# megaease/easevoice-trainer

Measured on AMD Instinct MI355X. Metric: audio-seconds/sec trained (s2), higher is better.
Workload: dtype bf16; 1 GPU; s2 SoVITS generator+discriminator GAN step, batch=16/GPU, 4 s 32 kHz clips (T=200 frames), configs/s2.json, random-init weights; global_batch=16, parallelism=dp1, launch=hip-graph replay (3 graphs/step)

## Files before the change

easevoice_trainer_amd/csrc/wn_layer.hip:

```cpp
#include "resunit_common.h"
#include "../../include/evt.h"
#include <type_traits>

namespace {

using namespace evt_ru;

struct WNP {
  const h16_t* x;
  const h16_t* w_in;
  const h16_t* w_rs;
  const float* b_in;
  const float* b_rs;
  const h16_t* g;
  const h16_t* acc_in;
  const int* lens;
  h16_t* x_in;
  h16_t* acts;
  h16_t* x_out;
  h16_t* acc_out;
  int nseq, L, tps;
};

__device__ __forceinline__ float sigmoid_f(float x) {
  return __builtin_amdgcn_rcpf(1.f + __builtin_amdgcn_exp2f(x * -1.4426950408889634f));
}
__device__ __forceinline__ float tanh_f(float x) { return fmaf(2.f, sigmoid_f(2.f * x), -1.f); }

__device__ __forceinline__ int wslot(int row, int slot) { return slot ^ (row & 7); }

__device__ __forceinline__ void unpack4(const u32x2 v, float (&o)[4]) {
  o[0] = h2f_lo(v[0]); o[1] = h2f_hi(v[0]);
  o[2] = h2f_lo(v[1]); o[3] = h2f_hi(v[1]);
}

template <int H, int K, int NT, int R, bool LAST>
__global__ __launch_bounds__(256, 1) void wn_layer_fwd(WNP p) {
  constexpr int PITCH = H * 2;
  constexpr int SPR = H / 8;
  constexpr int NCH = H / 32;
  constexpr int MT = H / 16 / 4;
  constexpr int P = 16 * NT;
  constexpr int HALO = (K - 1) / 2;
  constexpr int XROWS = P + K - 1;
  constexpr int NKA = NCH * K, NKB = NCH;
  constexpr int MA = 2 * MT;
  constexpr int MB = LAST ? MT : 2 * MT;
  static_assert(H % 64 == 0 && SPR % 8 == 0, "rows of whole 128-byte groups, M-tiles divisible by the four waves");
  extern __shared__ __attribute__((aligned(1024))) unsigned char smem[];
  unsigned char* xs = smem;
  unsigned char* acl = smem + ((XROWS + 7) & ~7) * PITCH;
  const int tid = threadIdx.x, lane = tid & 63, wm = __builtin_amdgcn_readfirstlane(tid >> 6);
  const int n = lane & 15, g = lane >> 4;
  const int seq = blockIdx.x / p.tps;
  const int q0 = (blockIdx.x - seq * p.tps) * P;
  const long sbase = (long)seq * p.L;

  u32x4 fa[R][MA];
  auto tileA = [&](int i) {
    return i < MT ? wm * MT + i : H / 16 + wm * MT + i - MT;
  };
  auto issue_a = [&](const h16_t* w, const int nk, const int ks, const int s, auto cnt) {
    constexpr int CNT = decltype(cnt)::value;
#pragma unroll
    for (int i = 0; i < CNT; ++i)
      fa[s][i] = *reinterpret_cast<const u32x4*>(w + ((long)(tileA(i) * nk + ks) * 64 + lane) * 8);
  };
  using CA = std::integral_constant<int, MA>;
  using CB = std::integral_constant<int, MB>;

  constexpr int NP = XROWS * SPR;
  constexpr int PER = (NP + 255) / 256;
  uint4 xv[PER];
#pragma unroll
  for (int u = 0; u < PER; ++u) {
    const int idx = u * 256 + tid;
    const int r = idx / SPR, sl = idx - r * SPR;
    const int pos = q0 - HALO + r;
    xv[u] = (idx < NP && pos >= 0 && pos < p.L) ? *reinterpret_cast<const uint4*>(p.x + (sbase + pos) * H + sl * 8)
                                                : make_uint4(0, 0, 0, 0);
  }
#pragma unroll
  for (int s = 0; s < R - 1 && s < NKA; ++s) issue_a(p.w_in, NKA, s, s, CA{});
  float bA0[MT][4], bA1[MT][4], bB0[MT][4], bB1[MT][4];
  u32x2 gA0[MT], gA1[MT], accp[MT][NT];
  const int len = p.lens ? p.lens[seq] : p.L;
#pragma unroll
  for (int i = 0; i < MT; ++i) {
    const int h = (wm * MT + i) * 16 + g * 4;
    const f32x4 z = {0.f, 0.f, 0.f, 0.f};
    const f32x4 a0 = p.b_in ? *reinterpret_cast<const f32x4*>(p.b_in + h) : z;
    const f32x4 a1 = p.b_in ? *reinterpret_cast<const f32x4*>(p.b_in + H + h) : z;
    const f32x4 c0 = p.b_rs ? *reinterpret_cast<const f32x4*>(p.b_rs + h) : z;
    const f32x4 c1 = (!LAST && p.b_rs) ? *reinterpret_cast<const f32x4*>(p.b_rs + H + h) : z;
#pragma unroll
    for (int r = 0; r < 4; ++r) { bA0[i][r] = a0[r]; bA1[i][r] = a1[r]; bB0[i][r] = c0[r]; bB1[i][r] = c1[r]; }
    gA0[i] = gA1[i] = u32x2{0u, 0u};
    if (p.g) {
      gA0[i] = *reinterpret_cast<const u32x2*>(p.g + (long)seq * 2 * H + h);
      gA1[i] = *reinterpret_cast<const u32x2*>(p.g + (long)seq * 2 * H + H + h);
    }
#pragma unroll
    for (int j = 0; j < NT; ++j) {
      const int pos = q0 + j * 16 + n;
      accp[i][j] = (p.acc_in && pos < p.L) ? *reinterpret_cast<const u32x2*>(p.acc_in + (sbase + pos) * H + h) : u32x2{0u, 0u};
    }
  }
#pragma unroll
  for (int u = 0; u < PER; ++u) {
    const int idx = u * 256 + tid;
    if (idx >= NP) continue;
    const int r = idx / SPR, sl = idx - r * SPR;
    *reinterpret_cast<uint4*>(xs + r * PITCH + wslot(r, sl) * 16) = xv[u];
  }
  __syncthreads();

  auto conv = [&](auto& acc, const h16_t* w, auto nk_c, auto taps_c, auto cnt, const unsigned char* rows) {
    constexpr int NK = decltype(nk_c)::value, TAPS = decltype(taps_c)::value, CNT = decltype(cnt)::value;
    u32x4 fb[NT];
    auto b_addr = [&](const int ks) {
      const int ch = ks / TAPS, tap = ks - ch * TAPS;
      const int row = n + tap;
      return rows + row * PITCH + wslot(row, ch * 4 + g) * 16;
    };
    {
      const unsigned char* b0 = b_addr(0);
#pragma unroll
      for (int j = 0; j < NT; ++j) {
        fb[j] = *reinterpret_cast<const u32x4*>(b0 + j * 16 * PITCH);
      }
    }
#pragma unroll
    for (int ks = 0; ks < NK; ++ks) {
      const int s = ks % R;
      if (ks + R - 1 < NK) issue_a(w, NK, ks + R - 1, (ks + R - 1) % R, cnt);
#pragma unroll
      for (int i = 0; i < CNT; ++i) tie(fa[s][i]);
      const unsigned char* nb = b_addr(ks + 1 < NK ? ks + 1 : ks);
#pragma unroll
      for (int j = 0; j < NT; ++j) {
        tie(fb[j]);
#pragma unroll
        for (int i = 0; i < CNT; ++i)
          acc[i][j] = EVT_MFMA_16x16x32(as_h8(fa[s][i]), as_h8(fb[j]), acc[i][j], 0, 0, 0);
        fb[j] = *reinterpret_cast<const u32x4*>(nb + j * 16 * PITCH);
      }
    }
  };

  {
    f32x4 acc[MA][NT];
#pragma unroll
    for (int i = 0; i < MA; ++i)
#pragma unroll
      for (int j = 0; j < NT; ++j) acc[i][j] = f32x4{0.f, 0.f, 0.f, 0.f};
    conv(acc, p.w_in, std::integral_constant<int, NKA>{}, std::integral_constant<int, K>{}, CA{}, xs);
#pragma unroll
    for (int s = 0; s < R - 1 && s < NKB; ++s) issue_a(p.w_rs, NKB, s, s, CB{});
#pragma unroll
    for (int i = 0; i < MT; ++i) {
      const int h = (wm * MT + i) * 16 + g * 4;
      float ga[4], gb[4];
      unpack4(gA0[i], ga);
      unpack4(gA1[i], gb);
#pragma unroll
      for (int j = 0; j < NT; ++j) {
        const int m = j * 16 + n;
        const int pos = q0 + m;
        h16_t xa[4], xb[4], o4[4];
#pragma unroll
        for (int r = 0; r < 4; ++r) {
          xa[r] = f2h(acc[i][j][r] + bA0[i][r]);
          xb[r] = f2h(acc[MT + i][j][r] + bA1[i][r]);
          const float a = h2f(xa[r]) + ga[r], b = h2f(xb[r]) + gb[r];
          o4[r] = f2h(tanh_f(a) * sigmoid_f(b));
        }
        *reinterpret_cast<uint2*>(acl + m * PITCH + wslot(m, h >> 3) * 16 + (h & 7) * 2) = *reinterpret_cast<uint2*>(o4);
        if (pos < p.L) {
          h16_t* xi = p.x_in + (sbase + pos) * 2 * H + h;
          *reinterpret_cast<uint2*>(xi) = *reinterpret_cast<uint2*>(xa);
          *reinterpret_cast<uint2*>(xi + H) = *reinterpret_cast<uint2*>(xb);
          *reinterpret_cast<uint2*>(p.acts + (sbase + pos) * H + h) = *reinterpret_cast<uint2*>(o4);
        }
      }
    }
  }
  __syncthreads();

  {
    f32x4 acc[MB][NT];
#pragma unroll
    for (int i = 0; i < MB; ++i)
#pragma unroll
      for (int j = 0; j < NT; ++j) acc[i][j] = f32x4{0.f, 0.f, 0.f, 0.f};
    conv(acc, p.w_rs, std::integral_constant<int, NKB>{}, std::integral_constant<int, 1>{}, CB{}, acl);
#pragma unroll
    for (int i = 0; i < MT; ++i) {
      const int h = (wm * MT + i) * 16 + g * 4;
#pragma unroll
      for (int j = 0; j < NT; ++j) {
        const int m = j * 16 + n;
        const int pos = q0 + m;
        if (pos >= p.L) continue;
        const bool live = pos < len;
        float ap[4];
        unpack4(accp[i][j], ap);
        h16_t o1[4], o2[4];
        if constexpr (LAST) {
#pragma unroll
          for (int r = 0; r < 4; ++r) {
            const float rs = h2f(f2h(acc[i][j][r] + bB0[i][r]));
            o2[r] = f2h(live ? ap[r] + rs : 0.f);
          }
        } else {
          float xo[4];
          const int xr = HALO + m;
          unpack4(*reinterpret_cast<const u32x2*>(xs + xr * PITCH + wslot(xr, h >> 3) * 16 + (h & 7) * 2), xo);
#pragma unroll
          for (int r = 0; r < 4; ++r) {
            const float r0 = h2f(f2h(acc[i][j][r] + bB0[i][r]));
            const float r1 = h2f(f2h(acc[MT + i][j][r] + bB1[i][r]));
            o1[r] = f2h(live ? xo[r] + r0 : 0.f);
            o2[r] = f2h(ap[r] + r1);
          }
          *reinterpret_cast<uint2*>(p.x_out + (sbase + pos) * H + h) = *reinterpret_cast<uint2*>(o1);
        }
        *reinterpret_cast<uint2*>(p.acc_out + (sbase + pos) * H + h) = *reinterpret_cast<uint2*>(o2);
      }
    }
  }
}

struct WNB {
  const h16_t* dx_next;
  const h16_t* dacc;
  const h16_t* x_in;
  const h16_t* g;
  const h16_t* w_rs;
  const h16_t* w_in;
  const int* lens;
  h16_t* drs;
  h16_t* dx_in;
  h16_t* dx;
  float* dg;
  int nseq, L, tps;
};

__device__ __forceinline__ int wslot2(int row, int slot) { return slot ^ ((row & 7) << 1); }

__device__ __forceinline__ float sum16(float v) {
  v += __shfl_xor(v, 1, 16);
  v += __shfl_xor(v, 2, 16);
  v += __shfl_xor(v, 4, 16);
  v += __shfl_xor(v, 8, 16);
  return v;
}

template <int H, int K, int NT, int R, bool LAST>
__global__ __launch_bounds__(256, 1) void wn_layer_bwd(WNB p) {
  constexpr int PB = H * 4;
  constexpr int SPRB = H / 4;
  constexpr int MT = H / 16 / 4;
  constexpr int P = 16 * NT;
  constexpr int HALO = (K - 1) / 2;
  constexpr int NT1 = NT + 1;
  constexpr int ROWS = P + 2 * HALO;
  constexpr int CIN1 = LAST ? H : 2 * H;
  constexpr int NK1 = CIN1 / 32, NK2 = (2 * H / 32) * K;
  static_assert(2 * HALO <= 16, "one extra position tile covers the halo");
  extern __shared__ __attribute__((aligned(1024))) unsigned char smem[];
  unsigned char* ds = smem;
  unsigned char* es = smem + 16 * NT1 * PB;
  const int tid = threadIdx.x, lane = tid & 63, wm = __builtin_amdgcn_readfirstlane(tid >> 6);
  const int n = lane & 15, g = lane >> 4;
  const int seq = blockIdx.x / p.tps;
  const int q0 = (blockIdx.x - seq * p.tps) * P;
  const long sbase = (long)seq * p.L;
  const int len = p.lens ? p.lens[seq] : p.L;

  u32x4 fa[R][MT];
  auto issue_a = [&](const h16_t* w, const int nk, const int ks, const int s) {
#pragma unroll
    for (int i = 0; i < MT; ++i)
      fa[s][i] = *reinterpret_cast<const u32x4*>(w + ((long)((wm * MT + i) * nk + ks) * 64 + lane) * 8);
  };

  constexpr int SPR1 = CIN1 / 8;
  constexpr int NP = ROWS * SPR1;
  constexpr int PER = (NP + 255) / 256;
  uint4 dv[PER];
#pragma unroll
  for (int u = 0; u < PER; ++u) {
    const int idx = u * 256 + tid;
    const int r = idx / SPR1, sl = idx - r * SPR1;
    const int pos = q0 - HALO + r;
    uint4 v = make_uint4(0, 0, 0, 0);
    if (idx < NP && pos >= 0 && pos < p.L) {
      if (LAST) {
        if (pos < len) v = *reinterpret_cast<const uint4*>(p.dacc + (sbase + pos) * H + sl * 8);
      } else if (sl < H / 8) {
        if (p.dx_next && pos < len) v = *reinterpret_cast<const uint4*>(p.dx_next + (sbase + pos) * H + sl * 8);
      } else {
        v = *reinterpret_cast<const uint4*>(p.dacc + (sbase + pos) * H + (sl - H / 8) * 8);
      }
    }
    dv[u] = v;
  }
#pragma unroll
  for (int s = 0; s < R - 1 && s < NK1; ++s) issue_a(p.w_rs, NK1, s, s);
  u32x2 xa[MT][NT1], xb[MT][NT1], ga[MT], gb[MT];
#pragma unroll
  for (int i = 0; i < MT; ++i) {
    const int h = (wm * MT + i) * 16 + g * 4;
    ga[i] = gb[i] = u32x2{0u, 0u};
    if (p.g) {
      ga[i] = *reinterpret_cast<const u32x2*>(p.g + (long)seq * 2 * H + h);
      gb[i] = *reinterpret_cast<const u32x2*>(p.g + (long)seq * 2 * H + H + h);
    }
#pragma unroll
    for (int j = 0; j < NT1; ++j) {
      const int m = j * 16 + n;
      const int pos = q0 - HALO + m;
      const bool in = m < ROWS && pos >= 0 && pos < p.L;
      xa[i][j] = in ? *reinterpret_cast<const u32x2*>(p.x_in + (sbase + pos) * 2 * H + h) : u32x2{0u, 0u};
      xb[i][j] = in ? *reinterpret_cast<const u32x2*>(p.x_in + (sbase + pos) * 2 * H + H + h) : u32x2{0u, 0u};
    }
  }
#pragma unroll
  for (int u = 0; u < PER; ++u) {
    const int idx = u * 256 + tid;
    if (idx >= NP) continue;
    const int r = idx / SPR1, sl = idx - r * SPR1;
    *reinterpret_cast<uint4*>(ds + r * PB + wslot2(r, sl) * 16) = dv[u];
    const int pos = q0 - HALO + r;
    if (r >= HALO && r < HALO + P && pos < p.L)
      *reinterpret_cast<uint4*>(p.drs + (sbase + pos) * CIN1 + sl * 8) = dv[u];
  }
  __syncthreads();

  auto conv = [&](auto& acc, const h16_t* w, auto nk_c, auto taps_c, auto nt_c, const unsigned char* rows) {
    constexpr int NK = decltype(nk_c)::value, TAPS = decltype(taps_c)::value, NTC = decltype(nt_c)::value;
    u32x4 fb[NTC];
    auto b_addr = [&](const int ks) {
      const int ch = ks / TAPS, tap = ks - ch * TAPS;
      const int row = n + tap;
      return rows + row * PB + wslot2(row, ch * 4 + g) * 16;
    };
    {
      const unsigned char* b0 = b_addr(0);
#pragma unroll
      for (int j = 0; j < NTC; ++j) fb[j] = *reinterpret_cast<const u32x4*>(b0 + j * 16 * PB);
    }
#pragma unroll
    for (int ks = 0; ks < NK; ++ks) {
      const int s = ks % R;
      if (ks + R - 1 < NK) issue_a(w, NK, ks + R - 1, (ks + R - 1) % R);
#pragma unroll
      for (int i = 0; i < MT; ++i) tie(fa[s][i]);
      const unsigned char* nb = b_addr(ks + 1 < NK ? ks + 1 : ks);
#pragma unroll
      for (int j = 0; j < NTC; ++j) {
        tie(fb[j]);
#pragma unroll
        for (int i = 0; i < MT; ++i)
          acc[i][j] = EVT_MFMA_16x16x32(as_h8(fa[s][i]), as_h8(fb[j]), acc[i][j], 0, 0, 0);
        fb[j] = *reinterpret_cast<const u32x4*>(nb + j * 16 * PB);
      }
    }
  };

  {
    f32x4 acc[MT][NT1];
#pragma unroll
    for (int i = 0; i < MT; ++i)
#pragma unroll
      for (int j = 0; j < NT1; ++j) acc[i][j] = f32x4{0.f, 0.f, 0.f, 0.f};
    conv(acc, p.w_rs, std::integral_constant<int, NK1>{}, std::integral_constant<int, 1>{}, std::integral_constant<int, NT1>{}, ds);
#pragma unroll
    for (int s = 0; s < R - 1 && s < NK2; ++s) issue_a(p.w_in, NK2, s, s);
#pragma unroll
    for (int i = 0; i < MT; ++i) {
      const int h = (wm * MT + i) * 16 + g * 4;
      float gaf[4], gbf[4], sa[4] = {0.f, 0.f, 0.f, 0.f}, sb[4] = {0.f, 0.f, 0.f, 0.f};
      unpack4(ga[i], gaf);
      unpack4(gb[i], gbf);
#pragma unroll
      for (int j = 0; j < NT1; ++j) {
        const int m = j * 16 + n;
        const int pos = q0 - HALO + m;
        const bool in = m < ROWS && pos >= 0 && pos < p.L;
        const bool own = in && m >= HALO && m < HALO + P;
        float xaf[4], xbf[4];
        unpack4(xa[i][j], xaf);
        unpack4(xb[i][j], xbf);
        h16_t oa[4], ob[4];
#pragma unroll
        for (int r = 0; r < 4; ++r) {
          const float d = h2f(f2h(acc[i][j][r]));
          const float t = tanh_f(xaf[r] + gaf[r]), sg = sigmoid_f(xbf[r] + gbf[r]);
          const float da = in ? d * sg * (1.f - t * t) : 0.f, db = in ? d * t * sg * (1.f - sg) : 0.f;
          oa[r] = f2h(da);
          ob[r] = f2h(db);
          if (own) { sa[r] += da; sb[r] += db; }
        }
        unsigned char* ep = es + m * PB;
        *reinterpret_cast<uint2*>(ep + wslot2(m, h >> 3) * 16 + (h & 7) * 2) = *reinterpret_cast<uint2*>(oa);
        *reinterpret_cast<uint2*>(ep + wslot2(m, (H + h) >> 3) * 16 + (h & 7) * 2) = *reinterpret_cast<uint2*>(ob);
        if (own) {
          h16_t* o = p.dx_in + (sbase + pos) * 2 * H + h;
          *reinterpret_cast<uint2*>(o) = *reinterpret_cast<uint2*>(oa);
          *reinterpret_cast<uint2*>(o + H) = *reinterpret_cast<uint2*>(ob);
        }
      }
      if (p.dg) {
#pragma unroll
        for (int r = 0; r < 4; ++r) {
          const float ta = sum16(sa[r]), tb = sum16(sb[r]);
          if (n == 0) {
            atomicAdd(p.dg + (long)seq * 2 * H + h + r, ta);
            atomicAdd(p.dg + (long)seq * 2 * H + H + h + r, tb);
          }
        }
      }
    }
  }
  __syncthreads();

  {
    f32x4 acc[MT][NT];
#pragma unroll
    for (int i = 0; i < MT; ++i)
#pragma unroll
      for (int j = 0; j < NT; ++j) acc[i][j] = f32x4{0.f, 0.f, 0.f, 0.f};
    conv(acc, p.w_in, std::integral_constant<int, NK2>{}, std::integral_constant<int, K>{}, std::integral_constant<int, NT>{}, es);
#pragma unroll
    for (int i = 0; i < MT; ++i) {
      const int h = (wm * MT + i) * 16 + g * 4;
#pragma unroll
      for (int j = 0; j < NT; ++j) {
        const int m = j * 16 + n;
        const int pos = q0 + m;
        if (pos >= p.L) continue;
        float dr[4] = {0.f, 0.f, 0.f, 0.f};
        if (!LAST) {
          const int r0 = HALO + m;
          unpack4(*reinterpret_cast<const u32x2*>(ds + r0 * PB + wslot2(r0, h >> 3) * 16 + (h & 7) * 2), dr);
        }
        h16_t o4[4];
#pragma unroll
        for (int r = 0; r < 4; ++r) o4[r] = f2h(acc[i][j][r] + dr[r]);
        *reinterpret_cast<uint2*>(p.dx + (sbase + pos) * H + h) = *reinterpret_cast<uint2*>(o4);
      }
    }
  }
}

__global__ __launch_bounds__(256) void frag_pack_kernel(const evt_frag_item* items) {
  const evt_frag_item it = items[blockIdx.y];
  const int nk = it.ktot / 32;
  const long pieces = (long)it.rows * it.ktot / 8;
  const uint4* src = reinterpret_cast<const uint4*>(it.src);
  uint4* dst = reinterpret_cast<uint4*>(it.dst);
  for (long pc = blockIdx.x * 256L + threadIdx.x; pc < pieces; pc += gridDim.x * 256L) {
    const int lane = (int)(pc & 63);
    const long ts = pc >> 6;
    const int tile = (int)(ts / nk), ks = (int)(ts - (long)tile * nk);
    dst[pc] = src[((long)(tile * 16 + (lane & 15)) * it.ktot + ks * 32 + (lane >> 4) * 8) / 8];
  }
}

template <int NT, int R, bool LAST>
int launch(WNP p, hipStream_t st) {
  constexpr int H = 192, K = 5, P = 16 * NT;
  p.tps = (p.L + P - 1) / P;
  const size_t lds = (size_t)(((P + K - 1 + 7) & ~7) + P) * H * 2;
  evt_set_last_tag("wn_layer_fwd<%s, %d, k%d, nt %d, ring %d%s>", EVT_HALF_NAME, H, K, NT, R, LAST ? ", last" : "");
  hipLaunchKernelGGL((wn_layer_fwd<H, K, NT, R, LAST>), dim3(p.nseq * p.tps), dim3(256), lds, st, p);
  return evt_check_launch();
}

template <int NT, int R, bool LAST>
int launch_b(WNB p, hipStream_t st) {
  constexpr int H = 192, K = 5, P = 16 * NT;
  p.tps = (p.L + P - 1) / P;
  const size_t lds = (size_t)2 * 16 * (NT + 1) * H * 4;
  static bool attr = false;
  if (!attr && lds > 64 * 1024) {
    if (hipFuncSetAttribute(reinterpret_cast<const void*>(&wn_layer_bwd<H, K, NT, R, LAST>),
                            hipFuncAttributeMaxDynamicSharedMemorySize, 160 * 1024) != hipSuccess)
      return EVT_ELAUNCH;
    attr = true;
  }
  evt_set_last_tag("wn_layer_bwd<%s, %d, k%d, nt %d, ring %d%s>", EVT_HALF_NAME, H, K, NT, R, LAST ? ", last" : "");
  hipLaunchKernelGGL((wn_layer_bwd<H, K, NT, R, LAST>), dim3(p.nseq * p.tps), dim3(256), lds, st, p);
  return evt_check_launch();
}

}

extern "C" {

int32_t evt_wn_layer_supported(int32_t dtype, int32_t H, int32_t k, int32_t dil) {
  return (dtype == EVT_DT_HALF && H == 192 && k == 5 && dil == 1) ? 1 : 0;
}

int evt_frag_pack(const evt_frag_item* items, int32_t nitems, void* stream) {
  if (!items || nitems <= 0) return EVT_EINVAL;
  evt_set_last_tag("frag_pack x%d", nitems);
  hipLaunchKernelGGL(frag_pack_kernel, dim3(32, nitems), dim3(256), 0, (hipStream_t)stream, items);
  return evt_check_launch();
}

int evt_wn_layer_fwd(int32_t dtype, const void* x, const void* w_in_frag, const float* b_in, const void* w_rs_frag,
                     const float* b_rs, const void* g, const void* acc_in, const int32_t* lens, void* x_in, void* acts,
                     void* x_out, void* acc_out, int32_t nseq, int32_t L, int32_t H, int32_t k, int32_t last, void* stream) {
  if (!evt_wn_layer_supported(dtype, H, k, 1)) return EVT_ENOTSUP;
  if (!x || !w_in_frag || !w_rs_frag || !x_in || !acts || !acc_out || (!last && !x_out) || nseq <= 0 || L <= 0) return EVT_EINVAL;
  WNP p{};
  p.x = (const h16_t*)x; p.w_in = (const h16_t*)w_in_frag; p.w_rs = (const h16_t*)w_rs_frag; p.b_in = b_in; p.b_rs = b_rs;
  p.g = (const h16_t*)g; p.acc_in = (const h16_t*)acc_in; p.lens = lens;
  p.x_in = (h16_t*)x_in; p.acts = (h16_t*)acts; p.x_out = (h16_t*)x_out; p.acc_out = (h16_t*)acc_out;
  p.nseq = nseq; p.L = L;
  hipStream_t st = (hipStream_t)stream;
  return last ? launch<1, 8, true>(p, st) : launch<1, 8, false>(p, st);
}

int evt_wn_layer_bwd_data(int32_t dtype, const void* dx_next, const void* dacc, const void* x_in, const void* g,
                          const void* w_rs_alt_frag, const void* w_in_alt_frag, const int32_t* lens, void* drs, void* dx_in,
                          void* dx, float* dg, int32_t nseq, int32_t L, int32_t H, int32_t k, int32_t last, void* stream) {
  if (!evt_wn_layer_supported(dtype, H, k, 1)) return EVT_ENOTSUP;
  if (!dacc || !x_in || !w_rs_alt_frag || !w_in_alt_frag || !drs || !dx_in || !dx || nseq <= 0 || L <= 0) return EVT_EINVAL;
  if (last && dx_next) return EVT_EINVAL;
  WNB p{};
  p.dx_next = (const h16_t*)dx_next; p.dacc = (const h16_t*)dacc; p.x_in = (const h16_t*)x_in; p.g = (const h16_t*)g;
  p.w_rs = (const h16_t*)w_rs_alt_frag; p.w_in = (const h16_t*)w_in_alt_frag; p.lens = lens;
  p.drs = (h16_t*)drs; p.dx_in = (h16_t*)dx_in; p.dx = (h16_t*)dx; p.dg = dg;
  p.nseq = nseq; p.L = L;
  hipStream_t st = (hipStream_t)stream;
  return last ? launch_b<1, 8, true>(p, st) : launch_b<1, 8, false>(p, st);
}

}
```

easevoice_trainer_amd/hip/wn.py:

```python
import torch

from . import conv as HC
from . import lib as L


class WNStackFn(torch.autograd.Function):
    @staticmethod
    def forward(ctx, x, g_lbh, lens, anchor, in_slots, rs_slots, hidden):
        n_layers, H = len(in_slots), hidden
        B, T, _ = x.shape
        if not x.is_contiguous() or x.size(2) != H or (g_lbh is not None and not g_lbh.is_contiguous()):
            raise L.EvtError("WN stack: contiguous [B, T, H] input and [n_layers, B, 2H] conditioning expected")
        dt = L.dt_of(x)
        rows = B * T
        saved = []
        out = None
        fused = FUSED_FORWARD and _layer_fused(dt, H, in_slots, rs_slots)
        frag_in, frag_rs = _frag_images(in_slots, rs_slots) if fused else (None, None)
        for i in range(n_layers):
            last = i == n_layers - 1
            if fused:
                mi, mr = in_slots[i].module, rs_slots[i].module
                x_in = torch.empty((B, T, 2 * H), dtype=x.dtype, device=x.device)
                acts = torch.empty((B, T, H), dtype=x.dtype, device=x.device)
                acc_out = torch.empty((B, T, H), dtype=x.dtype, device=x.device)
                x_out = None if last else torch.empty_like(acc_out)
                e0 = HC._t0()
                L.check(L.lib().evt_wn_layer_fwd(dt, L.ptr(x), L.ptr(frag_in[i]),
                                                 L.ptr(mi.bias.data if mi.bias is not None else None), L.ptr(frag_rs[i]),
                                                 L.ptr(mr.bias.data if mr.bias is not None else None),
                                                 L.ptr(g_lbh[i] if g_lbh is not None else None), L.ptr(out), L.ptr(lens),
                                                 L.ptr(x_in), L.ptr(acts), L.ptr(x_out), L.ptr(acc_out), B, T, H, mi.k,
                                                 int(last), L.stream_ptr()), "evt_wn_layer_fwd")
                if e0 is not None:
                    _t1_layer(e0, mi, mr, x)
                saved += [x, x_in, acts]
                x, out = x_out, acc_out
                continue
            x_in = HC._fwd(in_slots[i], x, None, 1.0, L.ACT_NONE, 1.0)
            acts = torch.empty((B, T, H), dtype=x.dtype, device=x.device)
            L.check(L.lib().evt_gated_act_fwd(dt, L.ptr(x_in), L.ptr(g_lbh[i] if g_lbh is not None else None), L.ptr(acts),
                                              B, T, H, L.stream_ptr()), "evt_gated_act_fwd")
            rs = HC._fwd(rs_slots[i], acts, None, 1.0, L.ACT_NONE, 1.0)
            acc_out = torch.empty((B, T, H), dtype=x.dtype, device=x.device)
            x_out = None if last else torch.empty_like(acc_out)
            L.check(L.lib().evt_wn_residual_fwd(dt, L.ptr(None if last else x), L.ptr(rs), L.ptr(out), L.ptr(lens), T,
                                                L.ptr(x_out), L.ptr(acc_out), rows, H, int(last),
                                                L.stream_ptr()), "evt_wn_residual_fwd")
            saved += [x, x_in, acts]
            x, out = x_out, acc_out
        ctx.save_for_backward(lens, g_lbh, *saved)
        ctx.cfg = (in_slots, rs_slots, H, B, T)
        return out

    @staticmethod
    def backward(ctx, dout):
        lens, g_lbh, *saved = ctx.saved_tensors
        in_slots, rs_slots, H, B, T = ctx.cfg
        n_layers = len(in_slots)
        dtype, dev = dout.dtype, dout.device
        dt = L.dt_code(dtype)
        rows = B * T
        dacc = dout.contiguous()
        dx_next = None
        dg32 = torch.zeros((n_layers, B, 2 * H), dtype=torch.float32, device=dev) if g_lbh is not None else None
        fused = FUSED_BACKWARD and _layer_fused(dt, H, in_slots, rs_slots)
        group = [] if (GROUP_WGRADS and HC.TRACE is None) else None

        def wgrad(*args):
            if group is None:
                HC._bwd_weight(*args)
                return
            group.append(args)
            if len(group) >= 2 * GROUP_LAYERS:
                HC._bwd_weight_group(list(group))
                group.clear()

        for i in reversed(range(n_layers)):
            last = i == n_layers - 1
            x, x_in, acts = saved[3 * i: 3 * i + 3]
            rs_w = H if last else 2 * H
            if fused:
                si, sr = in_slots[i], rs_slots[i]
                drs = torch.empty((B, T, rs_w), dtype=dtype, device=dev)
                dx_in = torch.empty((B, T, 2 * H), dtype=dtype, device=dev)
                dx = torch.empty((B, T, H), dtype=dtype, device=dev)
                e0 = HC._t0()
                L.check(L.lib().evt_wn_layer_bwd_data(dt, L.ptr(dx_next), L.ptr(dacc), L.ptr(x_in),
                                                      L.ptr(g_lbh[i] if g_lbh is not None else None),
                                                      L.ptr(sr.bank.frag(sr, "alt")), L.ptr(si.bank.frag(si, "alt")),
                                                      L.ptr(lens), L.ptr(drs), L.ptr(dx_in), L.ptr(dx),
                                                      L.ptr(dg32[i] if dg32 is not None else None), B, T, H, si.module.k,
                                                      int(last), L.stream_ptr()), "evt_wn_layer_bwd_data")
                if e0 is not None:
                    _t1_layer(e0, si.module, sr.module, x, "bwd_data")
                if last:
                    dacc = drs
                if sr.bank.weight_grads:
                    wgrad(sr, acts, drs, None, B, T, 1.0, L.ACT_NONE, 1.0)
                if si.bank.weight_grads:
                    wgrad(si, x, dx_in, None, B, T, 1.0, L.ACT_NONE, 1.0)
                dx_next = dx
                continue
            drs = torch.empty((B, T, rs_w), dtype=dtype, device=dev)
            dx_res = None if last else torch.empty((B, T, H), dtype=dtype, device=dev)
            L.check(L.lib().evt_wn_residual_bwd(dt, L.ptr(dx_next), L.ptr(dacc), L.ptr(lens), T, L.ptr(dx_res), L.ptr(drs),
                                                rows, H, int(last), L.stream_ptr()), "evt_wn_residual_bwd")
            if last:
                dacc = drs
            s = rs_slots[i]
            if s.bank.weight_grads:
                wgrad(s, acts, drs, None, B, T, 1.0, L.ACT_NONE, 1.0)
            dacts = HC._bwd_data(s, drs, None, acts, None, B, T, 1.0, L.ACT_NONE, 1.0)
            dx_in = torch.empty_like(x_in)
            L.check(L.lib().evt_gated_act_bwd(dt, L.ptr(x_in), L.ptr(g_lbh[i] if g_lbh is not None else None), L.ptr(dacts),
                                              L.ptr(dx_in), L.ptr(dg32[i] if dg32 is not None else None), B, T, H,
                                              L.stream_ptr()), "evt_gated_act_bwd")
            s = in_slots[i]
            if s.bank.weight_grads:
                wgrad(s, x, dx_in, None, B, T, 1.0, L.ACT_NONE, 1.0)
            need_dx = i > 0 or ctx.needs_input_grad[0]
            dx_next = HC._bwd_data(s, dx_in, None, x, dx_res, B, T, 1.0, L.ACT_NONE, 1.0) if need_dx else None
        if group:
            HC._bwd_weight_group(group)
        dg = dg32.to(g_lbh.dtype) if (dg32 is not None and ctx.needs_input_grad[1]) else None
        return dx_next, dg, None, None, None, None, None


FUSED_FORWARD = True
FUSED_BACKWARD = True
GROUP_WGRADS = True
GROUP_LAYERS = 2


def _layer_fused(dt, H, in_slots, rs_slots):
    bank = in_slots[0].bank
    cache = bank.__dict__.setdefault("_wn_fused", {})
    key = (id(in_slots[0]), len(in_slots), dt, H)
    ok = cache.get(key)
    if ok is None:
        ok = cache[key] = _layer_fused_check(dt, H, in_slots, rs_slots)
    return ok


def _layer_fused_check(dt, H, in_slots, rs_slots):
    n = len(in_slots)
    for i, (si, sr) in enumerate(zip(in_slots, rs_slots)):
        mi, mr = si.module, sr.module
        if not L.lib().evt_wn_layer_supported(dt, H, mi.k, mi.dil):
            return False
        if (mi.cin, mi.cout, mi.stride, mi.groups, mi.pad, mi.transposed) != (H, 2 * H, 1, 1, (mi.k - 1) // 2, False):
            return False
        if (mr.cin, mr.cout, mr.k, mr.stride, mr.groups, mr.pad, mr.transposed) != (H, H if i == n - 1 else 2 * H, 1, 1, 1, 0,
                                                                                    False):
            return False
    return True


def _frag_images(in_slots, rs_slots):
    bank = in_slots[0].bank
    return [bank.frag(s, "reg") for s in in_slots], [bank.frag(s, "reg") for s in rs_slots]


def _t1_layer(e0, mi, mr, x, kind="fwd"):
    e0, rf = e0
    e1 = torch.cuda.Event(enable_timing=True)
    e1.record()
    if rf is not None:
        rf.__exit__(None, None, None)
    n, ln, h = x.shape
    macs = n * ln * (mi.cin * mi.cout * mi.k + mr.cin * mr.cout)
    HC.TRACE.append((L.lib().evt_last_kernel_tag().decode(), kind, 2 * macs,
                     (7 * x.numel() + mi.v.numel() + mr.v.numel()) * 2, e0, e1,
                     f"WN layer {h}>{mi.cout}>{mr.cout} k{mi.k} n{n} L{ln}", mi))


def wn_stack(x, g_lbh, lens, in_layers, rs_layers, hidden):
    in_slots = tuple(m._slot for m in in_layers)
    rs_slots = tuple(m._slot for m in rs_layers)
    if any(s is None for s in in_slots + rs_slots):
        raise L.EvtError("WN stack before WeightBank.attach(); there is no eager fallback")
    return WNStackFn.apply(x, g_lbh, lens, in_slots[0].bank.anchor, in_slots, rs_slots, int(hidden))
```

easevoice_trainer_amd/module/models.py:

```python

import functools
import math
import os

import torch
from torch import nn
from torch.nn import functional as F

from ..hip import lib as L
from ..hip.conv import Add3ScaleFn, EvtConv1d, GatedActFn, mask_tail, res_stage, res_unit, resample_rows
from ..hip.enc import new_site, rel_self_attention, unbind_rows, wn_residual, wn_residual_last
from ..hip.frontend import RvqEncoder, ncl_to_nlc
from ..hip.wn import wn_stack
from . import commons
from .attentions import Encoder, MultiHeadAttention, PointwiseEvtConv, linear_rows, pointwise

LRELU_SLOPE = 0.1
N_SYMBOLS = 732


def get_padding(kernel_size, dilation=1):
    return (kernel_size * dilation - dilation) // 2


class _ComputeDtype:
    cd = torch.float32


class WeightNormPointwise(PointwiseEvtConv):

    def __init__(self, cin, cout):
        super().__init__(cin, cout, weight_norm=True)


class WN(nn.Module, _ComputeDtype):

    def __init__(self, hidden_channels, kernel_size, dilation_rate, n_layers, gin_channels=0, p_dropout=0):
        super().__init__()
        assert kernel_size % 2 == 1
        self.hidden_channels, self.n_layers, self.gin_channels = hidden_channels, n_layers, gin_channels
        self.in_layers = nn.ModuleList()
        self.res_skip_layers = nn.ModuleList()
        self.drop = nn.Dropout(p_dropout)
        if gin_channels != 0:
            self.cond_layer = WeightNormPointwise(gin_channels, 2 * hidden_channels * n_layers)
        for i in range(n_layers):
            dilation = dilation_rate ** i
            self.in_layers.append(EvtConv1d(hidden_channels, 2 * hidden_channels, kernel_size, dilation=dilation,
                                            padding=(kernel_size * dilation - dilation) // 2, weight_norm=True))
            rs = 2 * hidden_channels if i < n_layers - 1 else hidden_channels
            self.res_skip_layers.append(EvtConv1d(hidden_channels, rs, 1, weight_norm=True))

    def forward(self, x, x_mask, g=None, lens=None):
        H = self.hidden_channels
        if lens is None:
            lens = x_mask.sum(dim=(1, 2)).to(torch.int32)
        x = x.contiguous()
        if x.is_cuda and not (self.training and self.drop.p > 0):
            g_lbh = None
            if g is not None:
                g_lbh = self.cond_layer(g).to(x.dtype).view(g.size(0), self.n_layers, 2 * H).transpose(0, 1).contiguous()
            return wn_stack(x, g_lbh, lens, self.in_layers, self.res_skip_layers, H)
        gs = None
        if g is not None:
            g = self.cond_layer(g).to(x.dtype)
            gs = unbind_rows(g.view(g.size(0), self.n_layers, 2 * H).transpose(0, 1).contiguous())
        output = None
        for i in range(self.n_layers):
            x_in = self.in_layers[i](x)
            acts = self.drop(GatedActFn.apply(x_in, gs[i] if gs is not None else None))
            rs = self.res_skip_layers[i](acts)
            if i < self.n_layers - 1:
                x, output = wn_residual(x, rs, output, lens)
            else:
                output = wn_residual_last(rs, output, lens)
        return output


class PosteriorEncoder(nn.Module, _ComputeDtype):

    def __init__(self, in_channels, out_channels, hidden_channels, kernel_size, dilation_rate, n_layers,
                 gin_channels=0):
        super().__init__()
        self.out_channels = out_channels
        self.pre = pointwise(in_channels, hidden_channels)
        self.enc = WN(hidden_channels, kernel_size, dilation_rate, n_layers, gin_channels=gin_channels)
        self.proj = pointwise(hidden_channels, out_channels * 2)

    def forward(self, x, x_mask, g=None, eps=None, lens=None):
        if g is not None:
            g = g.detach()
        h = (self.pre(x) * x_mask).to(self.cd).contiguous()
        h = self.enc(h, x_mask, g=g, lens=lens)
        if h.is_cuda and lens is not None:
            from ..hip.enc import reparam

            stats = self.proj(h)
            if eps is None:
                eps = torch.randn((stats.size(0), stats.size(1), self.out_channels), dtype=torch.float32, device=h.device)
            return reparam(stats, eps, lens)
        stats = self.proj(h) * x_mask
        m, logs = torch.split(stats.float(), self.out_channels, dim=-1)
        if eps is None:
            eps = torch.randn_like(m)
        z = (m + eps * torch.exp(logs)) * x_mask
        return z, m, logs


class ResidualCouplingLayer(nn.Module, _ComputeDtype):

    def __init__(self, channels, hidden_channels, kernel_size, dilation_rate, n_layers, p_dropout=0, gin_channels=0,
                 mean_only=False):
        super().__init__()
        assert channels % 2 == 0
        self.half_channels, self.mean_only = channels // 2, mean_only
        self.pre = pointwise(self.half_channels, hidden_channels)
        self.enc = WN(hidden_channels, kernel_size, dilation_rate, n_layers, p_dropout=p_dropout,
                      gin_channels=gin_channels)
        self.post = pointwise(hidden_channels, self.half_channels * (2 - mean_only))
        self.post.weight.data.zero_()
        self.post.bias.data.zero_()

    def forward(self, x, x_mask, g=None, reverse=False, lens=None):
        x0, x1 = torch.split(x, [self.half_channels] * 2, dim=-1)
        h = (self.pre(x0) * x_mask).to(self.cd).contiguous()
        h = self.enc(h, x_mask, g=g, lens=lens)
        stats = (self.post(h) * x_mask).float()
        if self.mean_only:
            x1 = stats + x1 * x_mask if not reverse else (x1 - stats) * x_mask
            return torch.cat([x0, x1], dim=-1)
        m, logs = torch.split(stats, [self.half_channels] * 2, dim=-1)
        if not reverse:
            x1 = m + x1 * torch.exp(logs) * x_mask
        else:
            x1 = (x1 - m) * torch.exp(-logs) * x_mask
        return torch.cat([x0, x1], dim=-1)

    def forward_flip(self, x, x0c, x_mask, mask_cd, g, lens, want_next):
        from ..hip.enc import coupling_flip

        if x0c is None:
            x0c = x[..., :self.half_channels]
        h = (self.pre(x0c) * mask_cd).contiguous()
        h = self.enc(h, x_mask, g=g, lens=lens)
        return coupling_flip(x, self.post(h), lens, want_next)


class Flip(nn.Module):
    def forward(self, x, *args, **kwargs):
        return torch.flip(x, [-1])


class ResidualCouplingBlock(nn.Module):

    def __init__(self, channels, hidden_channels, kernel_size, dilation_rate, n_layers, n_flows=4, gin_channels=0):
        super().__init__()
        self.flows = nn.ModuleList()
        for _ in range(n_flows):
            self.flows.append(ResidualCouplingLayer(channels, hidden_channels, kernel_size, dilation_rate, n_layers,
                                                    gin_channels=gin_channels, mean_only=True))
            self.flows.append(Flip())

    def forward(self, x, x_mask, g=None, reverse=False, lens=None):
        if (not reverse and x.is_cuda and lens is not None and x.dtype == torch.float32
                and all(f.mean_only for f in self.flows[0::2])):
            x0c = None
            n = len(self.flows) // 2
            mask_cd = x_mask.to(self.flows[0].cd)
            for i in range(n):
                x, x0c = self.flows[2 * i].forward_flip(x, x0c, x_mask, mask_cd, g, lens, want_next=i + 1 < n)
            return x
        flows = self.flows if not reverse else reversed(self.flows)
        for flow in flows:
            x = flow(x, x_mask, g=g, reverse=reverse, lens=lens)
        return x


class MRTE(nn.Module):

    def __init__(self, content_enc_channels=192, hidden_size=512, out_channels=192, n_heads=4):
        super().__init__()
        self.cross_attention = MultiHeadAttention(hidden_size, hidden_size, n_heads)
        self.c_pre = pointwise(content_enc_channels, hidden_size)
        self.text_pre = pointwise(content_enc_channels, hidden_size)
        self.c_post = pointwise(hidden_size, out_channels)

    def forward(self, ssl_enc, ssl_mask, text, text_mask, ge, ssl_lens, text_lens):
        ssl_enc = self.c_pre(ssl_enc * ssl_mask)
        text_enc = self.text_pre(text * text_mask)
        x = self.cross_attention(ssl_enc * ssl_mask, text_enc * text_mask, ssl_lens, text_lens) + ssl_enc
        if ge is not None:
            x = x + ge.unsqueeze(1)
        return self.c_post(x * ssl_mask)


class TextEncoder(nn.Module, _ComputeDtype):

    def __init__(self, out_channels, hidden_channels, filter_channels, n_heads, n_layers, kernel_size, p_dropout,
                 latent_channels=192, version="v2"):
        super().__init__()
        self.out_channels = out_channels
        self.ssl_proj = pointwise(768, hidden_channels)
        self.encoder_ssl = Encoder(hidden_channels, filter_channels, n_heads, n_layers // 2, kernel_size, p_dropout)
        self.encoder_text = Encoder(hidden_channels, filter_channels, n_heads, n_layers, kernel_size, p_dropout)
        self.text_embedding = nn.Embedding(N_SYMBOLS, hidden_channels)
        self.mrte = MRTE()
        self.encoder2 = Encoder(hidden_channels, filter_channels, n_heads, n_layers // 2, kernel_size, p_dropout)
        self.proj = pointwise(hidden_channels, out_channels * 2)

    def forward(self, y, y_mask, text, text_mask, ge, y_lengths=None, text_lengths=None, speed=1, out_lens=None):
        yl = (y_lengths if y_lengths is not None else y_mask.sum(dim=(1, 2))).to(torch.int32)
        tl = (text_lengths if text_lengths is not None else text_mask.sum(dim=(1, 2))).to(torch.int32)
        y = self.ssl_proj(y * y_mask)
        y = self.encoder_ssl(y, y_mask, self.cd, lengths=yl)
        t = self.text_embedding(text)
        t = self.encoder_text(t, text_mask, self.cd, lengths=tl)
        y = self.mrte(y, y_mask, t, text_mask, ge, yl, tl)
        y = self.encoder2(y, y_mask, self.cd, lengths=yl)
        if speed != 1:
            n = int(y.size(1) / speed) + 1
            y = F.interpolate(y.transpose(1, 2).float(), size=n, mode="linear").transpose(1, 2).to(y.dtype).contiguous()
            y_mask = F.interpolate(y_mask.transpose(1, 2), size=n, mode="nearest").transpose(1, 2).contiguous()
        if out_lens is not None:
            if speed != 1:
                raise L.EvtError("TextEncoder.forward: out_lens (per-row resampling) goes with speed == 1")
            ol = torch.as_tensor(out_lens, dtype=torch.int32).reshape(-1)
            n = int(ol.max())
            ol = ol.to(y.device)
            y = resample_rows(y.contiguous(), yl.contiguous(), ol, n, self.proj)
            y_mask = commons.sequence_mask(ol, n).unsqueeze(-1).to(y_mask.dtype)
        stats = (self.proj(y) * y_mask).float()
        m, logs = torch.split(stats, self.out_channels, dim=-1)
        return (y, m, logs) if speed == 1 and out_lens is None else (y, m, logs, y_mask)


class LinearNorm(nn.Module):
    def __init__(self, cin, cout, bias=True):
        super().__init__()
        if not bias:
            raise L.EvtError("LinearNorm without a bias is not used by the style encoder (modules.py:521-545)")
        self.fc = linear_rows(cin, cout)

    def forward(self, x):
        return self.fc(x)


class Mish(nn.Module):
    def forward(self, x):
        return x * torch.tanh(F.softplus(x))


class ConvNorm(nn.Module):
    def __init__(self, cin, cout, kernel_size):
        super().__init__()
        self.conv = EvtConv1d(cin, cout, kernel_size, padding=(kernel_size - 1) // 2)

    def forward(self, x):
        return self.conv(x)


class Conv1dGLU(nn.Module, _ComputeDtype):

    def __init__(self, in_channels, out_channels, kernel_size, dropout):
        super().__init__()
        self.out_channels = out_channels
        self.conv1 = ConvNorm(in_channels, 2 * out_channels, kernel_size)
        self.dropout = nn.Dropout(dropout)
        self._site = new_site()

    def forward(self, x):
        residual = x
        h = self.conv1(x.to(self.cd).contiguous())
        if h.is_cuda:
            from ..hip.enc import glu_dropout_res

            return glu_dropout_res(h, residual, self.dropout.p if self.training else 0.0, self._site)
        x1, x2 = torch.split(h, self.out_channels, dim=-1)
        return residual + self.dropout(x1 * torch.sigmoid(x2))

    def forward_rows(self, x, lens):
        from ..hip.enc import glu_res_rows

        return glu_res_rows(self.conv1(x.to(self.cd).contiguous()), x, lens)


class StyleAttention(nn.Module):

    def __init__(self, n_head, d_model, d_k, d_v, dropout=0.0):
        super().__init__()
        self.n_head, self.d_k, self.d_v = n_head, d_k, d_v
        self.w_qs = linear_rows(d_model, n_head * d_k)
        self.w_ks = linear_rows(d_model, n_head * d_k)
        self.w_vs = linear_rows(d_model, n_head * d_v)
        if d_k != d_v:
            raise L.EvtError("the fused attention core takes one head width (d_k == d_v, as the style encoder has it)")
        self.temperature = float(d_model) ** 0.5
        self.fc = linear_rows(n_head * d_v, d_model)
        self.dropout = nn.Dropout(dropout)
        self.attn_dropout = nn.Dropout(dropout)
        self._site = new_site()

    def forward(self, x, lens):
        p = self.attn_dropout.p if self.training else 0.0
        cd = self.w_qs._slot.bank.dtype if self.w_qs._slot is not None else x.dtype
        x = x.to(cd).contiguous()
        out = rel_self_attention(x, self.w_qs, self.w_ks, self.w_vs, None, None, lens, self.n_head, None, p, self._site,
                                 scale=1.0 / self.temperature)
        return self.dropout(self.fc(out)) + x


class MelStyleEncoder(nn.Module):

    def __init__(self, n_mel_channels=80, style_hidden=128, style_vector_dim=256, style_kernel_size=5, style_head=2,
                 dropout=0.1):
        super().__init__()
        self.spectral = nn.Sequential(LinearNorm(n_mel_channels, style_hidden), Mish(), nn.Dropout(dropout),
                                      LinearNorm(style_hidden, style_hidden), Mish(), nn.Dropout(dropout))
        self.temporal = nn.Sequential(Conv1dGLU(style_hidden, style_hidden, style_kernel_size, dropout),
                                      Conv1dGLU(style_hidden, style_hidden, style_kernel_size, dropout))
        self.slf_attn = StyleAttention(style_head, style_hidden, style_hidden // style_head,
                                       style_hidden // style_head, dropout)
        self.fc = LinearNorm(style_hidden, style_vector_dim)
        self._sites = (new_site(), new_site())
        self.mask_beyond_collate = False

    def _spectral(self, x):
        sp = self.spectral
        if not x.is_cuda:
            return sp(x)
        from ..hip.enc import mish_dropout

        x = mish_dropout(sp[0](x), sp[2].p if self.training else 0.0, self._sites[0])
        return mish_dropout(sp[3](x), sp[5].p if self.training else 0.0, self._sites[1], torch.float32)

    def forward(self, x, x_mask, lens=None):
        pad = x_mask.squeeze(-1) == 0
        if lens is None:
            lens = x_mask.sum(dim=(1, 2))
        x = self._spectral(x)
        if self.mask_beyond_collate:
            t_ref = 2 * (torch.div(lens.max(), 2, rounding_mode="floor") + 1)
            live = (torch.arange(x.size(1), device=x.device) < t_ref).to(x.dtype).view(1, -1, 1)
            x = x * live
        x = self.temporal(x)
        x = x.masked_fill(pad.unsqueeze(-1), 0)
        x = self.slf_attn(x, lens.to(torch.int32))
        x = self.fc(x)
        n = (~pad).sum(dim=1, keepdim=True)
        return x.masked_fill(pad.unsqueeze(-1), 0).sum(dim=1) / n

    @torch.no_grad()
    def forward_rows(self, x, lens):
        if self.training:
            raise L.EvtError("MelStyleEncoder.forward_rows is the inference form: call eval() first")
        if not x.is_cuda:
            raise L.EvtError("MelStyleEncoder.forward_rows runs on the library's kernels: the input must be on the GPU")
        from ..hip.enc import mean_rows, mish_rows

        sp = self.spectral
        slot = self.fc.fc._slot
        bank = slot.bank if slot is not None else None
        pin = bank is not None and L.is_half(bank.dtype) and bank.impl == L.IMPL_AUTO
        if pin:
            bank.impl = L.IMPL_IGEMM
        try:
            x = mish_rows(sp[0](x), lens)
            x = mish_rows(sp[3](x), lens, torch.float32)
            for glu in self.temporal:
                x = glu.forward_rows(x, lens)
            x = self.slf_attn(x, lens)
            return mean_rows(self.fc(x), lens)
        finally:
            if pin:
                bank.impl = L.IMPL_AUTO


class _Codebook(nn.Module):
    KMEANS_ITERS = 50
    KMEANS_SAMPLES = 500

    def __init__(self, dim, codebook_size):
        super().__init__()
        self.codebook_size = codebook_size
        self.register_buffer("inited", torch.Tensor([False]))
        self.register_buffer("cluster_size", torch.zeros(codebook_size))
        self.register_buffer("embed", torch.zeros(codebook_size, dim))
        self.register_buffer("embed_avg", torch.zeros(codebook_size, dim))

    @torch.no_grad()
    def init_embed_(self, data):
        samples = data[:self.KMEANS_SAMPLES].float()
        n, K = samples.shape[0], self.codebook_size
        if n >= K:
            idx = torch.randperm(n, device=samples.device)[:K]
        else:
            idx = torch.randint(0, n, (K,), device=samples.device)
        means = samples[idx]
        bins = None
        for _ in range(self.KMEANS_ITERS):
            buckets = torch.cat([(-((samples[i:i + 50, None, :] - means[None]) ** 2).sum(dim=-1)).max(dim=-1).indices
                                 for i in range(0, n, 50)])
            bins = torch.bincount(buckets, minlength=K)
            zero = bins == 0
            new_means = torch.zeros_like(means)
            new_means.scatter_add_(0, buckets[:, None].expand(-1, samples.shape[1]), samples)
            new_means = new_means / bins.masked_fill(zero, 1)[:, None]
            means = torch.where(zero[:, None], means, new_means)
        self.embed.copy_(means)
        self.embed_avg.copy_(means)
        self.cluster_size.copy_(bins.to(self.cluster_size.dtype))
        self.inited.fill_(1.0)


class _VQLayer(nn.Module):
    def __init__(self, dim, codebook_size):
        super().__init__()
        self._codebook = _Codebook(dim, codebook_size)


class _RVQ(nn.Module):
    def __init__(self, dim, codebook_size, n_q):
        super().__init__()
        self.layers = nn.ModuleList([_VQLayer(dim, codebook_size) for _ in range(n_q)])


class ResidualVectorQuantizer(nn.Module):

    def __init__(self, dimension=256, n_q=8, bins=1024):
        super().__init__()
        self.n_q, self.dimension, self.bins = n_q, dimension, bins
        self.vq = _RVQ(dimension, bins, n_q)

    def ensure_init(self, h):
        if getattr(self, "_inited_ok", False):
            return
        cb = self.vq.layers[0]._codebook
        if not bool(cb.inited.cpu().item()):
            cb.init_embed_(h.reshape(-1, h.size(-1)))
            import torch.distributed as dist
            if dist.is_available() and dist.is_initialized() and dist.get_world_size() > 1:
                for buf in (cb.embed, cb.embed_avg, cb.cluster_size, cb.inited):
                    dist.broadcast(buf, src=0)
        self._inited_ok = True

    @torch.no_grad()
    def decode(self, codes):
        q = None
        for layer, ind in zip(self.vq.layers, codes):
            e = F.embedding(ind, layer._codebook.embed)
            q = e if q is None else q + e
        return q


def rvq_encode(enc, quantizer, ssl, rep):
    h = enc.project(ssl)
    quantizer.ensure_init(h)
    q, codes = enc.lookup(h, rep)
    return q, codes.unsqueeze(0)


class ResBlock1(nn.Module):

    def __init__(self, channels, kernel_size=3, dilation=(1, 3, 5)):
        super().__init__()
        self.convs1 = nn.ModuleList([
            EvtConv1d(channels, channels, kernel_size, dilation=d, padding=get_padding(kernel_size, d), weight_norm=True)
            for d in dilation])
        self.convs2 = nn.ModuleList([
            EvtConv1d(channels, channels, kernel_size, dilation=1, padding=get_padding(kernel_size, 1), weight_norm=True)
            for _ in dilation])

    def forward(self, x, lens=None, mul=1):
        for c1, c2 in zip(self.convs1, self.convs2):
            x = res_unit(x, c1, c2, LRELU_SLOPE) if lens is None else res_unit(x, c1, c2, LRELU_SLOPE, lens, mul)
        return x


class Generator(nn.Module, _ComputeDtype):

    def __init__(self, initial_channel, resblock, resblock_kernel_sizes, resblock_dilation_sizes, upsample_rates,
                 upsample_initial_channel, upsample_kernel_sizes, gin_channels=0):
        super().__init__()
        if str(resblock) != "1":
            raise L.EvtError("only ResBlock1 (configs/s2.json resblock='1') is implemented")
        self.num_kernels, self.num_upsamples = len(resblock_kernel_sizes), len(upsample_rates)
        self.conv_pre = EvtConv1d(initial_channel, upsample_initial_channel, 7, padding=3)
        self.ups = nn.ModuleList()
        for i, (u, k) in enumerate(zip(upsample_rates, upsample_kernel_sizes)):
            self.ups.append(EvtConv1d(upsample_initial_channel // (2 ** i), upsample_initial_channel // (2 ** (i + 1)),
                                      k, stride=u, padding=(k - u) // 2, transposed=True, weight_norm=True))
        self.resblocks = nn.ModuleList()
        ch = upsample_initial_channel
        for i in range(len(self.ups)):
            ch = upsample_initial_channel // (2 ** (i + 1))
            for k, d in zip(resblock_kernel_sizes, resblock_dilation_sizes):
                self.resblocks.append(ResBlock1(ch, k, tuple(d)))
        self.conv_post = EvtConv1d(ch, 1, 7, padding=3, bias=False)
        if gin_channels != 0:
            self.cond = pointwise(gin_channels, upsample_initial_channel)

    def forward(self, x, g=None, lens=None):
        x = x.to(self.cd).contiguous()
        if lens is not None:
            x = mask_tail(x.clone(), lens, 1, self.conv_pre)
        x = self.conv_pre(x)
        if g is not None:
            x = (x + self.cond(g).unsqueeze(1)).to(self.cd)
        mul = 1
        if lens is not None:
            x = mask_tail(x.contiguous(), lens, 1, self.conv_pre)
        for i in range(self.num_upsamples):
            x = self.ups[i](x, in_slope=LRELU_SLOPE)
            blocks = [self.resblocks[i * self.num_kernels + j] for j in range(self.num_kernels)]
            if lens is not None:
                mul *= self.ups[i].stride
            if x.is_cuda:
                xs = res_stage(x, blocks, LRELU_SLOPE, 1.0 / self.num_kernels, lens, mul)
                if xs is not None:
                    x = xs
                    continue
            if lens is not None:
                x = mask_tail(x, lens, mul, self.ups[i])
                blocks = [functools.partial(b, lens=lens, mul=mul) for b in blocks]
            lane = None
            if x.is_cuda and len(blocks) == 3:
                from ..hip.disc import _On, dec_lane

                lane = dec_lane(x.device)
            if lane is not None:
                main = torch.cuda.current_stream(x.device)
                lane.wait_stream(main)
                with _On(lane):
                    r0, r1 = blocks[0](x), blocks[1](x)
                x.record_stream(lane)
                r2 = blocks[2](x)
                main.wait_stream(lane)
                r0.record_stream(main)
                r1.record_stream(main)
                rs = [r0, r1, r2]
            else:
                rs = [b(x) for b in blocks]
            while len(rs) < 3:
                rs.append(None)
            x = Add3ScaleFn.apply(rs[0], rs[1], rs[2], 1.0 / self.num_kernels, self)
        return self.conv_post(x, in_slope=0.01, out_act=L.ACT_TANH)


class DiscriminatorP(nn.Module, _ComputeDtype):

    def __init__(self, period, kernel_size=5, stride=3, use_spectral_norm=False):
        super().__init__()
        if use_spectral_norm:
            raise L.EvtError("spectral_norm discriminators are not used by configs/s2.json")
        self.period = period
        chans = [1, 32, 128, 512, 1024, 1024]
        self.convs = nn.ModuleList([
            EvtConv1d(chans[i], chans[i + 1], kernel_size, stride=(stride if i < 4 else 1),
                      padding=get_padding(kernel_size, 1), weight_norm=True, kdims=2) for i in range(5)])
        self.conv_post = EvtConv1d(1024, 1, 3, padding=1, weight_norm=True, kdims=2)

    def prepare(self, x):
        n, t = x.shape
        p = self.period
        if t % p != 0:
            x = F.pad(x.unsqueeze(1), (0, p - (t % p)), "reflect").squeeze(1)
            t = x.size(1)
        return x.view(n, t // p, p).transpose(1, 2).reshape(n * p, t // p, 1).to(self.cd).contiguous()

    def plan(self):
        convs = list(self.convs) + [self.conv_post]
        return (tuple(c._slot for c in convs),
                tuple([(L.ACT_LRELU, LRELU_SLOPE)] * len(self.convs) + [(L.ACT_NONE, 1.0)]))

    def forward(self, x):
        return self.forward_prepared(self.prepare(x))

    def forward_prepared(self, x):
        n = x.size(0) // self.period
        fmap = []
        for l in self.convs:
            x = l(x, out_act=L.ACT_LRELU, out_slope=LRELU_SLOPE)
            fmap.append(x)
        x = self.conv_post(x)
        fmap.append(x)
        return x.view(n, -1), fmap


class DiscriminatorS(nn.Module, _ComputeDtype):

    def __init__(self, use_spectral_norm=False):
        super().__init__()
        if use_spectral_norm:
            raise L.EvtError("spectral_norm discriminators are not used by configs/s2.json")
        spec = [(1, 16, 15, 1, 1, 7), (16, 64, 41, 4, 4, 20), (64, 256, 41, 4, 16, 20), (256, 1024, 41, 4, 64, 20),
                (1024, 1024, 41, 4, 256, 20), (1024, 1024, 5, 1, 1, 2)]
        self.convs = nn.ModuleList([EvtConv1d(ci, co, k, stride=s, groups=g, padding=p, weight_norm=True)
                                    for ci, co, k, s, g, p in spec])
        self.conv_post = EvtConv1d(1024, 1, 3, padding=1, weight_norm=True)

    def prepare(self, x):
        return x.unsqueeze(-1).to(self.cd).contiguous()

    def plan(self):
        convs = list(self.convs) + [self.conv_post]
        return (tuple(c._slot for c in convs),
                tuple([(L.ACT_LRELU, LRELU_SLOPE)] * len(self.convs) + [(L.ACT_NONE, 1.0)]))

    def forward(self, x):
        return self.forward_prepared(self.prepare(x))

    def forward_prepared(self, x):
        fmap = []
        for l in self.convs:
            x = l(x, out_act=L.ACT_LRELU, out_slope=LRELU_SLOPE)
            fmap.append(x)
        x = self.conv_post(x)
        fmap.append(x)
        return x.view(x.size(0), -1), fmap


class MultiPeriodDiscriminator(nn.Module):

    def __init__(self, use_spectral_norm=False):
        super().__init__()
        periods = [2, 3, 5, 7, 11]
        self.discriminators = nn.ModuleList([DiscriminatorS(use_spectral_norm)] +
                                            [DiscriminatorP(p, use_spectral_norm=use_spectral_norm) for p in periods])

    def periods(self):
        return tuple(getattr(d, "period", 1) for d in self.discriminators)

    def _prepared(self, y, y2=None):
        if y.is_cuda:
            from ..hip.disc import MPDFoldFn, mpd_fold

            cd = self.discriminators[0].cd
            if y2 is None and y.requires_grad:
                return list(MPDFoldFn.apply(y, self.periods(), cd))
            if y2 is None or not (y.requires_grad or y2.requires_grad):
                return mpd_fold(self.periods(), cd, y, y2)
        x = y if y2 is None else torch.cat([y.float(), y2.float()], dim=0)
        return [d.prepare(x.float()) for d in self.discriminators]

    def forward_single(self, y):
        y = y.reshape(y.size(0), -1)
        outs, fmaps = [], []
        for d, x in zip(self.discriminators, self._prepared(y)):
            o, f = d.forward_prepared(x)
            outs.append(o)
            fmaps.append(f)
        return outs, fmaps

    def generator_losses(self, y, y_hat):
        from ..hip.disc import MPDGenLossFn

        n = y.size(0)
        plan = tuple(d.plan() for d in self.discriminators)
        if any(s is None for slots, _ in plan for s in slots):
            raise L.EvtError("MultiPeriodDiscriminator used before WeightBank.attach(); there is no eager fallback")
        anchor = plan[0][0][0].bank.anchor
        out = MPDGenLossFn.apply(anchor, plan, self.periods(), y_hat.reshape(n, -1).contiguous(),
                                 y.reshape(n, -1).detach().contiguous())
        return out[0], out[1], list(out[2:])

    def forward_batched(self, y, y_hat):
        n = y.size(0)
        xs = self._prepared(y.reshape(n, -1), y_hat.reshape(n, -1))
        if not y.is_cuda:
            return [d.forward_prepared(x)[0] for d, x in zip(self.discriminators, xs)]
        from ..hip.disc import _On, _branches

        bank = self.discriminators[0].convs[0]._slot.bank if self.discriminators[0].convs[0]._slot is not None else None
        lanes, sides = _branches(y.device, len(self.discriminators)) if (bank is not None and bank.defer_n > 0) \
            else ([None] * len(self.discriminators), [])
        main = torch.cuda.current_stream(y.device) if sides else None
        for st in sides:
            st.wait_stream(main)
        outs = []
        for d, x, lane in zip(self.discriminators, xs, lanes):
            with _On(lane):
                o = d.forward_prepared(x)[0]
            if lane is not None:
                x.record_stream(lane)
                o.record_stream(main)
            outs.append(o)
        for st in sides:
            main.wait_stream(st)
        return outs

    def forward(self, y, y_hat):
        n = y.size(0)
        y_d_rs, y_d_gs, fmap_rs, fmap_gs = [], [], [], []
        for d, x in zip(self.discriminators, self._prepared(y.reshape(n, -1), y_hat.reshape(n, -1))):
            o, f = d.forward_prepared(x)
            y_d_rs.append(o[:n])
            y_d_gs.append(o[n:])
            fmap_rs.append([t[: t.size(0) // 2] for t in f])
            fmap_gs.append([t[t.size(0) // 2:] for t in f])
        return y_d_rs, y_d_gs, fmap_rs, fmap_gs


class SynthesizerTrn(nn.Module, _ComputeDtype):

    def __init__(self, spec_channels, segment_size, inter_channels, hidden_channels, filter_channels, n_heads,
                 n_layers, kernel_size, p_dropout, resblock, resblock_kernel_sizes, resblock_dilation_sizes,
                 upsample_rates, upsample_initial_channel, upsample_kernel_sizes, n_speakers=0, gin_channels=0,
                 use_sdp=True, semantic_frame_rate=None, freeze_quantizer=None, version="v2", **kwargs):
        super().__init__()
        self.spec_channels, self.segment_size, self.inter_channels = spec_channels, segment_size, inter_channels
        self.gin_channels, self.version = gin_channels, version
        self.upsample_rates = upsample_rates
        self.sampling_rate = 32000
        self.enc_p = TextEncoder(inter_channels, hidden_channels, filter_channels, n_heads, n_layers, kernel_size,
                                 p_dropout, version=version)
        self.dec = Generator(inter_channels, resblock, resblock_kernel_sizes, resblock_dilation_sizes, upsample_rates,
                             upsample_initial_channel, upsample_kernel_sizes, gin_channels=gin_channels)
        self.enc_q = PosteriorEncoder(spec_channels, inter_channels, hidden_channels, 5, 1, 16,
                                      gin_channels=gin_channels)
        self.flow = ResidualCouplingBlock(inter_channels, hidden_channels, 5, 1, 4, gin_channels=gin_channels)
        self.ref_enc = MelStyleEncoder(spec_channels if version == "v1" else 704, style_vector_dim=gin_channels)
        ssl_dim = 768
        assert semantic_frame_rate in ["25hz", "50hz"]
        self.semantic_frame_rate = semantic_frame_rate
        if semantic_frame_rate == "25hz":
            self.ssl_proj = nn.Conv1d(ssl_dim, ssl_dim, 2, stride=2)
        else:
            self.ssl_proj = nn.Conv1d(ssl_dim, ssl_dim, 1, stride=1)
        self.quantizer = ResidualVectorQuantizer(dimension=ssl_dim, n_q=1, bins=1024)
        self.freeze_quantizer = freeze_quantizer
        self.split_backward = False
        self._cut = None
        self._cut2 = None

    def _rvq(self):
        enc = getattr(self, "_rvq_enc", None)
        cb = self.quantizer.vq.layers[0]._codebook
        if enc is None or enc.bank.device != cb.embed.device:
            k = 2 if self.semantic_frame_rate == "25hz" else 1
            enc = RvqEncoder(lambda: self.ssl_proj.weight, lambda: self.ssl_proj.bias, lambda: cb.embed,
                             cb.embed.size(1), cb.codebook_size, k, k, cb.embed.device)
            object.__setattr__(self, "_rvq_enc", enc)
        return enc

    def _quantize(self, ssl):
        with torch.no_grad(), torch.autocast("cuda", enabled=False):
            return rvq_encode(self._rvq(), self.quantizer, ssl, 2 if self.semantic_frame_rate == "25hz" else 1)

    @torch.no_grad()
    def extract_latent(self, x):
        _q, codes = self._quantize(x)
        return codes.transpose(0, 1)

    @torch.no_grad()
    def extract_latent_rows(self, hs, frames):
        from ..hip import feat as HF

        cb = self.quantizer.vq.layers[0]._codebook
        w, bias, embed = self.ssl_proj.weight, self.ssl_proj.bias, cb.embed
        if self.semantic_frame_rate != "25hz":
            raise L.EvtError("extract_latent_rows serves the 25 Hz quantizer (ssl_proj with k = 2, stride 2)")
        if not torch.is_tensor(hs) or hs.dim() != 3:
            raise L.EvtError("extract_latent_rows: hidden states [B, Tmax, 768] expected")
        if hs.size(2) != embed.size(1):
            raise L.EvtError(f"extract_latent_rows: features of width {hs.size(2)}, the quantizer takes {embed.size(1)}")
        if hs.device != embed.device:
            raise L.EvtError(f"extract_latent_rows: features on {hs.device}, the model on {embed.device}")
        frames = [int(t) for t in (frames.reshape(-1).tolist() if torch.is_tensor(frames) else frames)]
        if len(frames) != hs.size(0):
            raise L.EvtError(f"extract_latent_rows: {len(frames)} frame counts for {hs.size(0)} rows")
        stamp = tuple((t.data_ptr(), t._version) for t in (w, bias, embed, cb.inited))
        cache = getattr(self, "_rows_cache", None)
        if cache is None or cache[0] != stamp:
            if not bool(cb.inited.cpu().item()):
                raise L.EvtError("extract_latent_rows: the codebook is not initialised (load a trained quantizer first)")
            al = lambda t: t if t.data_ptr() % 16 == 0 else t.clone()
            e = al(embed.detach().float().contiguous())
            cache = (stamp, HF.make_proj_image(w), al(bias.detach().float().contiguous()), e, HF.rvq_norms(e))
            object.__setattr__(self, "_rows_cache", cache)
        _stamp, image, b32, e32, ee = cache
        codes, _off = HF.semantic_codes_rows(hs.contiguous(), frames, image, b32, e32, ee)
        return list(torch.split(codes, [t // 2 for t in frames]))

    @torch.no_grad()
    def decode(self, codes, text, refer, noise_scale=0.5, speed=1, noise=None, style=None):
        amp = self.cd in (torch.bfloat16, torch.float16)
        with torch.autocast("cuda", dtype=self.cd if amp else torch.bfloat16, enabled=amp):
            ges = []
            for r in ([] if style is not None else refer if isinstance(refer, (list, tuple)) else [refer]):
                r_cl = r.transpose(1, 2)
                r_cl = r_cl if self.version == "v1" else r_cl[..., :704]
                ges.append(self.ref_enc(r_cl, torch.ones(r_cl.size(0), r_cl.size(1), 1, device=r.device)))
            ge = torch.stack(ges, 0).mean(0) if style is None else self._given_style(style, refer, codes.size(1), codes.device)
            B, Tc = codes.size(1), codes.size(2)
            T = Tc * 2 if self.semantic_frame_rate == "25hz" else Tc
            y_lengths = torch.full((B,), T, dtype=torch.long, device=codes.device)
            text_lengths = torch.full((B,), text.size(-1), dtype=torch.long, device=text.device)
            quantized = self.quantizer.decode(codes)
            if self.semantic_frame_rate == "25hz":
                quantized = quantized.repeat_interleave(2, dim=1)
            y_mask = torch.ones(B, T, 1, device=codes.device)
            text_mask = torch.ones(B, text.size(1), 1, device=text.device)
            enc = self.enc_p(quantized, y_mask, text, text_mask, ge, y_lengths, text_lengths, speed=speed)
            if speed != 1:
                _x, m_p, logs_p, y_mask = enc
                y_lengths = torch.full((B,), y_mask.size(1), dtype=torch.long, device=codes.device)
            else:
                _x, m_p, logs_p = enc
            if noise is None:
                noise = torch.randn(B, m_p.size(2), m_p.size(1), device=m_p.device)
            eps = noise[:, :, :m_p.size(1)].transpose(1, 2).to(m_p.dtype)
            z_p = m_p + eps * torch.exp(logs_p) * noise_scale
            ym = y_mask.to(self.cd)
            z = self.flow(z_p, ym, g=ge, reverse=True, lens=y_lengths.to(torch.int32))
            o = self.dec(z * ym, g=ge)
        return o.transpose(1, 2)

    def _style(self, refer):
        ges = []
        for r in (refer if isinstance(refer, (list, tuple)) else [refer]):
            r_cl = r.transpose(1, 2)
            r_cl = r_cl if self.version == "v1" else r_cl[..., :704]
            ges.append(self.ref_enc(r_cl, torch.ones(r_cl.size(0), r_cl.size(1), 1, device=r.device)))
        return torch.stack(ges, 0).mean(0)

    @torch.no_grad()
    def style_rows(self, spec_cl, lens):
        if spec_cl.dim() != 3 or spec_cl.dtype != torch.float32:
            raise L.EvtError(f"style_rows takes fp32 spectrograms [B, Tmax, bins] (channels-last), got {spec_cl.dtype} {tuple(spec_cl.shape)}")
        bins = spec_cl.size(2) if self.version == "v1" else 704
        if spec_cl.size(2) < bins or (self.version == "v1" and bins != self.spec_channels):
            raise L.EvtError(f"style_rows: the style encoder takes {bins} bins, the spectrograms have {spec_cl.size(2)}")
        if not torch.is_tensor(lens):
            lens = torch.tensor([int(v) for v in lens], dtype=torch.int32).to(spec_cl.device)
        lens = lens.to(torch.int32).contiguous()
        x = spec_cl if spec_cl.size(2) == bins else spec_cl[..., :bins].contiguous()
        amp = self.cd in (torch.bfloat16, torch.float16)
        with torch.autocast("cuda", dtype=self.cd if amp else torch.bfloat16, enabled=amp):
            return self.ref_enc.forward_rows(x, lens)

    def _given_style(self, style, refer, B, dev):
        if refer is not None:
            raise L.EvtError("decode: give either the reference spectrogram(s) `refer` or a precomputed `style`, not both")
        if not torch.is_tensor(style) or style.dim() != 2 or style.size(1) != self.gin_channels or style.size(0) not in (1, B):
            raise L.EvtError(f"decode: style must be [1, {self.gin_channels}] (shared) or [{B}, {self.gin_channels}] (one per "
                             f"row), got {tuple(style.shape) if torch.is_tensor(style) else type(style)}")
        if style.device != dev:
            raise L.EvtError(f"decode: style lives on {style.device}, the batch on {dev}")
        ge = style.to(torch.float32)
        return ge.contiguous() if ge.size(0) == B else ge.expand(B, -1).contiguous()

    @torch.no_grad()
    def decode_batch(self, codes, code_lens, text, text_lens, refer, noise_scale=0.5, noise=None, speed=1, out_rate=None,
                     out_format=None, interval=0.0, style=None):
        dev = codes.device
        if out_format is not None or out_rate is not None:
            from ..hip import audio

            out_rate = self.sampling_rate if out_rate is None else out_rate
            out_format = "float32" if out_format is None else out_format
            if out_format not in audio.FORMATS:
                raise L.EvtError(f"decode_batch: out_format must be one of {sorted(audio.FORMATS)}, got {out_format!r}")
            audio.rate_ratio(self.sampling_rate, out_rate)
        elif interval:
            raise L.EvtError("decode_batch: interval goes with out_rate / out_format (the packed output)")
        if codes.dim() != 3 or codes.size(0) != 1 or text.dim() != 2 or text.size(0) != codes.size(1):
            raise L.EvtError(f"decode_batch takes codes [1, B, Tc] and text [B, Tt], got {tuple(codes.shape)} and {tuple(text.shape)}")
        B, Tc = codes.size(1), codes.size(2)
        code_lens = torch.as_tensor(code_lens, dtype=torch.long).reshape(-1)
        text_lens = torch.as_tensor(text_lens, dtype=torch.long).reshape(-1)
        cl, tl = [int(v) for v in code_lens.tolist()], [int(v) for v in text_lens.tolist()]
        if len(cl) != B or len(tl) != B or min(cl) < 1 or max(cl) > Tc or min(tl) < 1 or max(tl) > text.size(1):
            raise L.EvtError(f"decode_batch: code_lens / text_lens must hold {B} lengths in [1, {Tc}] / [1, {text.size(1)}]")
        f = 2 if self.semantic_frame_rate == "25hz" else 1
        T = Tc * f
        if torch.is_tensor(speed):
            speed = speed.tolist()
        speeds = [float(v) for v in speed] if isinstance(speed, (list, tuple)) else [float(speed)] * B
        if len(speeds) != B:
            raise L.EvtError(f"decode_batch: speed holds {len(speeds)} values for {B} rows")
        for b, v in enumerate(speeds):
            if not (math.isfinite(v) and v > 0):
                raise L.EvtError(f"decode_batch: speed of row {b} is {v}, it must be finite and > 0")
        out_len = None if all(v == 1 for v in speeds) else [n * f if v == 1 else int(n * f / v) + 1 for n, v in zip(cl, speeds)]
        if out_len is not None and noise is not None and (noise.dim() != 3 or noise.size(0) not in (1, B)
                                                           or noise.size(2) < max(out_len)):
            raise L.EvtError(f"decode_batch: noise must be [{B}, inter, >= {max(out_len)}] at these speeds (a table of "
                             f"batch 1 is shared by the rows), got {tuple(noise.shape)}")
        amp = self.cd in (torch.bfloat16, torch.float16)
        with torch.autocast("cuda", dtype=self.cd if amp else torch.bfloat16, enabled=amp):
            per_row = isinstance(refer, (list, tuple)) and len(refer) == B
            if style is not None:
                ge = self._given_style(style, refer, B, dev)
            elif per_row:
                seen = {}
                for r in refer:
                    if id(r) not in seen:
                        seen[id(r)] = self._style(r)
                ge = torch.cat([seen[id(r)] for r in refer], 0)
            else:
                ge = self._style(refer)
                if ge.size(0) != 1:
                    raise L.EvtError("decode_batch: a shared reference is one spectrogram [1, spec, Tr] (or a list of them)")
                ge = ge.expand(B, -1).contiguous()
            y_lengths = (code_lens * f).to(dev)
            text_lengths = text_lens.to(dev)
            quantized = self.quantizer.decode(codes)
            if f == 2:
                quantized = quantized.repeat_interleave(2, dim=1)
            y_mask = commons.sequence_mask(y_lengths, T).unsqueeze(-1).to(torch.float32)
            text_mask = commons.sequence_mask(text_lengths, text.size(1)).unsqueeze(-1).to(torch.float32)
            if out_len is None:
                _x, m_p, logs_p = self.enc_p(quantized, y_mask, text, text_mask, ge, y_lengths, text_lengths)
                frames = [n * f for n in cl]
            else:
                _x, m_p, logs_p, y_mask = self.enc_p(quantized, y_mask, text, text_mask, ge, y_lengths, text_lengths,
                                                     out_lens=out_len)
                frames, T = out_len, max(out_len)
                y_lengths = torch.tensor(out_len, dtype=torch.long).to(dev)
            if noise is None:
                noise = torch.randn(B, m_p.size(2), m_p.size(1), device=m_p.device)
            eps = noise[:, :, :m_p.size(1)].transpose(1, 2).to(m_p.dtype)
            z_p = m_p + eps * torch.exp(logs_p) * noise_scale
            ym = y_mask.to(self.cd)
            lens32 = y_lengths.to(torch.int32)
            z = self.flow(z_p, ym, g=ge, reverse=True, lens=lens32)
            o = self.dec(z * ym, g=ge, lens=lens32)
        up = o.size(1) // T
        if out_format is not None:
            return audio.resample_pack(o, frames, up, self.sampling_rate, out_rate, out_format, interval=interval,
                                       lens_dev=lens32, owner=self.dec)
        return [o[b, :frames[b] * up, 0] for b in range(B)]

    def forward(self, ssl, y, y_lengths, text, text_lengths, eps=None, ids_slice=None):
        dev = y.device
        T = y.size(2)
        y_mask = commons.sequence_mask(y_lengths, T).unsqueeze(-1).to(torch.float32)
        text_mask = commons.sequence_mask(text_lengths, text.size(1)).unsqueeze(-1).to(torch.float32)
        amp = self.cd in (torch.bfloat16, torch.float16)
        with torch.autocast("cuda", dtype=self.cd if amp else torch.bfloat16, enabled=amp):
            lens32 = y_lengths.to(torch.int32)
            y_cl = ncl_to_nlc(y.float(), self.enc_q.pre.cin, self.cd)
            ref_in = y_cl[..., :self.spec_channels] if self.version == "v1" else y_cl[..., :704]
            split = self.split_backward and torch.is_grad_enabled()
            lane = None
            if y.is_cuda and not split:
                from ..hip.disc import _On, enc_lane

                lane = enc_lane(dev)
            if lane is not None and os.environ.get("EVT_QUANT_LANE", "1") != "0":
                main = torch.cuda.current_stream(dev)
                lane.wait_stream(main)
                with _On(lane):
                    quantized, _codes = self._quantize(ssl)
                ssl.record_stream(lane)
                ge = self.ref_enc(ref_in * y_mask.to(self.cd), y_mask, lens32)
            else:
                ge = self.ref_enc(ref_in * y_mask.to(self.cd), y_mask, lens32)
                quantized, _codes = self._quantize(ssl)
            if lane is not None:
                main = torch.cuda.current_stream(dev)
                lane.wait_stream(main)
                with _On(lane):
                    x, m_p, logs_p = self.enc_p(quantized, y_mask, text, text_mask, ge, y_lengths, text_lengths)
                for t in (quantized, y_mask, text, text_mask, ge, y_lengths, text_lengths):
                    t.record_stream(lane)
            else:
                x, m_p, logs_p = self.enc_p(quantized, y_mask, text, text_mask, ge, y_lengths, text_lengths)
            eps_cl = eps.transpose(1, 2) if eps is not None else None
            ym = y_mask.to(self.cd)
            ge_fq = ge
            if split:
                ge_fq = ge.detach().requires_grad_(True)
                m_p_cut, logs_p_cut = m_p.detach().requires_grad_(True), logs_p.detach().requires_grad_(True)
                self._cut2 = ((ge, ge_fq), (m_p, m_p_cut), (logs_p, logs_p_cut))
                m_p, logs_p = m_p_cut, logs_p_cut
            z, m_q, logs_q = self.enc_q(y_cl, ym, g=ge_fq, eps=eps_cl, lens=lens32)
            z_p = self.flow(z, ym, g=ge_fq, lens=lens32)
            if ids_slice is None:
                z_slice, ids_slice = commons.rand_slice_segments(z, y_lengths, self.segment_size)
            else:
                z_slice = commons.slice_segments(z, ids_slice, self.segment_size)
            if split:
                z_cut, ge_cut = z_slice.detach().requires_grad_(True), ge.detach().requires_grad_(True)
                self._cut = ((z_slice, z_cut), (ge, ge_cut))
                o = self.dec(z_cut, g=ge_cut)
            else:
                o = self.dec(z_slice, g=ge)
            if lane is not None:
                main.wait_stream(lane)
                for t in (x, m_p, logs_p, quantized):
                    t.record_stream(main)
        commit_loss = torch.zeros((), device=dev)
        tr = lambda t: t.transpose(1, 2)
        y_mask_ncl = y_mask.transpose(1, 2)
        return (o.transpose(1, 2), commit_loss, ids_slice, y_mask_ncl, y_mask_ncl,
                (tr(z), tr(z_p), tr(m_p), tr(logs_p), tr(m_q), tr(logs_q)), tr(quantized))
```

include/evt.h:

```cpp
#ifndef EVT_H
#define EVT_H
#include <stddef.h>
#include <stdint.h>

#ifdef __cplusplus
extern "C" {
#endif
#pragma GCC visibility push(default)

#define EVT_DT_F32 0
#define EVT_DT_BF16 1
#define EVT_DT_F16 2
#define EVT_ACT_NONE 0
#define EVT_ACT_LRELU 1
#define EVT_ACT_TANH 2
#define EVT_IMPL_AUTO 0
#define EVT_IMPL_NAIVE 1
#define EVT_IMPL_IGEMM 2

const char* evt_version(void);
int32_t evt_half_dtype(void);
void evt_debug_kernel_tags(int32_t enable);
const char* evt_last_kernel_tag(void);

#define EVT_WS_NONE 0
#define EVT_WS_MEL 1
#define EVT_WS_ATTN_BWD 2
#define EVT_WS_MHA_BWD 3
#define EVT_WS_MASKED_KL 4
int64_t evt_workspace_bytes(int32_t op, const int64_t* dims, int32_t ndims);

typedef struct evt_conv1d_params {
  int32_t dtype;
  int32_t nseq;
  int32_t lin;
  int32_t cin, cout;
  int32_t k, stride, pad, dil, groups;
  int32_t transposed;
  float in_slope;
  int32_t out_act;
  float out_slope;
  int32_t impl;
} evt_conv1d_params;

int32_t evt_conv1d_wants_plain_dy(const evt_conv1d_params* c);

int32_t evt_conv1d_wants_plain_x(const evt_conv1d_params* c);

int32_t evt_conv1d_lout(const evt_conv1d_params* p);

typedef struct evt_wlayout {
  int32_t d0, d1, k, stride;
  int32_t reg_ck, reg_nchunk, reg_kp;
  int32_t alt_ck, alt_nchunk, alt_kp, alt_nphase;
  int64_t reg_elems, alt_elems;
} evt_wlayout;
int evt_conv1d_layout(const evt_conv1d_params* p, evt_wlayout* out);

typedef struct evt_wprep_item {
  const float* v;
  const float* g;
  void* reg;
  void* alt;
  const float* dw;
  float* dv;
  float* dg;
  evt_wlayout lay;
  int32_t dtype;
  int32_t src_d1;
  const float* dw_extra;
  int64_t dw_part_stride;
  const float* db_part;
  float* db;
  const int32_t* used;
} evt_wprep_item;
int evt_wn_fold_multi(const evt_wprep_item* items, const int32_t* row_index, int32_t nrows, void* stream);
int evt_wn_fold_groups(const evt_wprep_item* items, const int32_t* group_index, int32_t ngroups, void* stream);
int evt_wn_grad_multi(const evt_wprep_item* items, const int32_t* row_index, int32_t nrows, void* stream);

int evt_conv1d_fwd(const evt_conv1d_params* p, const void* x, const void* w_reg, const void* w_alt,
                   const float* bias, const void* res, void* y, void* stream);

int evt_conv1d_bwd_data(const evt_conv1d_params* p, const void* dy, const void* y, const void* w_reg,
                        const void* w_alt, const void* x, const void* dx_add, void* dx, void* stream);

int evt_conv1d_bwd_weight(const evt_conv1d_params* p, const void* x, const void* dy, const void* y,
                          float* dw, float* dbias, void* stream);

typedef struct evt_wgrad_parts {
  float* dw_extra;
  int64_t part_stride;
  float* db_part;
  int32_t* used_dev;
  int32_t parts;
  int32_t prev_used;
  int32_t used;
  int32_t dirty0;
  float* ws;
  int64_t ws_floats;
} evt_wgrad_parts;
int evt_conv1d_bwd_weight_parts(const evt_conv1d_params* p, const void* x, const void* dy, const void* y,
                                float* dw, float* dbias, evt_wgrad_parts* sp, void* stream);

#define EVT_WGRAD_GROUP_MAX 16
typedef struct evt_wgrad_member {
  const evt_conv1d_params* p;
  const void* x;
  const void* dy;
  const void* y;
  float* dw;
  float* dbias;
  evt_wgrad_parts* sp;
} evt_wgrad_member;
int evt_conv1d_bwd_weight_group(const evt_wgrad_member* members, int32_t n, void* stream);

typedef struct evt_wgrad_plan {
  int64_t tiles;
  int32_t stages;
  int32_t min_stages;
  int32_t parts;
  int32_t launch;
  int32_t nsplit;
  int32_t per;
} evt_wgrad_plan;
int evt_wgrad_group_plan(evt_wgrad_plan* members, int32_t n, int64_t target);

typedef struct evt_resunit_params {
  int32_t dtype, nseq, L, C, k, dil;
  float slope;
} evt_resunit_params;
int32_t evt_resunit_supported(const evt_resunit_params* p);
int evt_resunit_fwd(const evt_resunit_params* p, const void* x, const void* w1_reg, const void* w2_reg, const float* b1,
                    const float* b2, void* xa, void* mid_a, void* y, void* stream);

typedef struct evt_resunit_fwd_job {
  evt_resunit_params p;
  const void* x; const void* w1_reg; const void* w2_reg; const float* b1; const float* b2;
  void* xa; void* mid_a; void* y;
} evt_resunit_fwd_job;
int evt_resunit_fwd_multi(const evt_resunit_fwd_job* jobs, int32_t njobs, void* stream);

int evt_resunit_fwd_multi_lens(const evt_resunit_fwd_job* jobs, int32_t njobs, const int32_t* lens, int32_t mul,
                               void* stream);

int32_t evt_resunit_bwd_supported(const evt_resunit_params* p, int32_t with_weight_grads);
int64_t evt_resunit_bwd_ws_floats(const evt_resunit_params* p);
int evt_resunit_bwd(const evt_resunit_params* p, const void* dy, float dy_scale, const void* xa, const void* mid_a,
                    const void* w1_alt, const void* w2_alt, void* dx, void* dmid, float* dw1, float* dw2, float* db1,
                    float* db2, float* ws, int64_t ws_floats, void* stream);
typedef struct evt_resunit_bwd_job {
  evt_resunit_params p;
  float dy_scale;
  const void* dy; const void* xa; const void* mid_a; const void* w1_alt; const void* w2_alt;
  void* dx; void* dmid;
  float* dw1; float* dw2; float* db1; float* db2;
} evt_resunit_bwd_job;
int evt_resunit_bwd_multi(const evt_resunit_bwd_job* jobs, int32_t njobs, float* ws, int64_t ws_floats, void* stream);

int32_t evt_resunit_wide_supported(const evt_resunit_params* p);
int evt_resunit_wide_fwd(const evt_resunit_params* p, const void* x, const void* w1_reg, const void* w2_reg, const float* b1,
                         const float* b2, void* xa, void* mid_a, void* y, void* stream);
int evt_resunit_wide_fwd_lens(const evt_resunit_params* p, const void* x, const void* w1_reg, const void* w2_reg,
                              const float* b1, const float* b2, void* xa, void* mid_a, void* y, const int32_t* lens,
                              int32_t mul, void* stream);
int evt_resunit_wide_bwd_data(const evt_resunit_params* p, const void* dy, float dy_scale, const void* xa, const void* mid_a,
                              const void* w1_alt, const void* w2_alt, void* dmid, void* dx, void* stream);

typedef struct evt_frag_item {
  const void* src;
  void* dst;
  int32_t rows, ktot;
} evt_frag_item;
int evt_frag_pack(const evt_frag_item* items, int32_t nitems, void* stream);
int evt_wn_layer_bwd_data(int32_t dtype, const void* dx_next, const void* dacc, const void* x_in, const void* g,
                          const void* w_rs_alt_frag, const void* w_in_alt_frag, const int32_t* lens, void* drs, void* dx_in,
                          void* dx, float* dg, int32_t nseq, int32_t L, int32_t H, int32_t k, int32_t last, void* stream);
int32_t evt_wn_layer_supported(int32_t dtype, int32_t H, int32_t k, int32_t dil);
int evt_wn_layer_fwd(int32_t dtype, const void* x, const void* w_in_frag, const float* b_in, const void* w_rs_frag,
                     const float* b_rs, const void* g, const void* acc_in, const int32_t* lens, void* x_in, void* acts,
                     void* x_out, void* acc_out, int32_t nseq, int32_t L, int32_t H, int32_t k, int32_t last, void* stream);

int evt_add3_scale(int32_t dtype, const void* a, const void* b, const void* c, float scale, void* out,
                   int64_t n, void* stream);

int evt_mask_tail(int32_t dtype, void* x, const int32_t* lens, int32_t mul, int32_t nseq, int32_t L, int32_t C,
                  void* stream);

int evt_resample_rows(int32_t dtype, const void* x, const int32_t* in_lens, const int32_t* out_lens, int32_t nseq,
                      int32_t Lin, int32_t Lout, int32_t C, void* y, void* stream);

#define EVT_RESAMPLE_ZEROS 64
#define EVT_RESAMPLE_TILE 2048
#define EVT_PCM_F32 0
#define EVT_PCM_S16 1
int evt_resample_pack_rows(int32_t dtype, const void* x, const int32_t* lens, int32_t mul, int32_t nseq, int32_t L,
                           int32_t up, int32_t down, const float* table, int32_t J, int32_t out_format, void* out,
                           int64_t out_elems, const int64_t* out_off, int32_t gap, void* stream);

int evt_leaky_relu(int32_t dtype, const void* x, float slope, void* out, int64_t n, void* stream);

int evt_dact_mul(int32_t dtype, const void* dy, const void* y, int32_t act_kind, float slope, void* out, int64_t n,
                 void* stream);

int evt_gated_act_fwd(int32_t dtype, const void* xin, const void* g, void* acts, int32_t nseq, int32_t len,
                      int32_t H, void* stream);
int evt_gated_act_bwd(int32_t dtype, const void* xin, const void* g, const void* dacts, void* dxin, float* dg,
                      int32_t nseq, int32_t len, int32_t H, void* stream);


int evt_mel_fwd(const float* wav, const float* window, const float* mel_basis, float* spec_out, float* mel_out,
                float* ws_spec_re_im, int32_t nseq, int32_t wav_len, int32_t n_fft, int32_t hop, int32_t n_mels,
                void* stream);
int evt_mel_bwd(const float* dmel, const float* window, const float* mel_basis, const float* ws_spec_re_im,
                float* dwav, int32_t nseq, int32_t wav_len, int32_t n_fft, int32_t hop, int32_t n_mels, void* stream);
int64_t evt_mel_workspace_floats(int32_t nseq, int32_t wav_len, int32_t n_fft, int32_t hop, int32_t n_mels);

int evt_ref_spec_rows(const float* x, const int32_t* lens, int32_t nseq, int32_t N, const float* window, int32_t n_fft,
                      int32_t hop, int32_t bins, float* out, float* peak, void* stream);

int evt_ncl_to_nlc(int32_t dtype, const float* src, void* dst, int32_t B, int32_t C, int32_t T, int32_t Cp, void* stream);

int evt_rvq_norms(const float* embed, float* ee, int32_t K, int32_t D, void* stream);
int evt_rvq_select(const float* h, const float* dots, const float* embed, const float* ee, int64_t* codes, float* q_out,
                   int32_t N, int32_t D, int32_t K, int32_t rep, void* stream);

int evt_spec_to_mel(const float* spec, const float* basis, const int64_t* starts, float* out, int32_t B, int32_t F,
                    int32_t T, int32_t M, int32_t nfr, void* stream);

typedef struct evt_seg { const void* a; const void* b; void* da; int64_t n; float scale; int32_t pad_; } evt_seg;
int evt_l1_multi_fwd(int32_t dtype, const evt_seg* segs, int32_t nseg, float* out, void* stream);
int evt_l1_multi_bwd(int32_t dtype, const evt_seg* segs, int32_t nseg, const float* dloss, void* stream);
int evt_lsgan_multi_fwd(int32_t dtype, const evt_seg* segs, int32_t nseg, float target, float* out, void* stream);
int evt_lsgan_multi_bwd(int32_t dtype, const evt_seg* segs, int32_t nseg, float target, const float* dloss,
                        void* stream);

typedef struct evt_kl_params {
  int32_t B, T, C, time_inner;
  int32_t dt_z_p, dt_logs_q, dt_m_p, dt_logs_p;
} evt_kl_params;
int evt_masked_kl_fwd(const evt_kl_params* p, const void* z_p, const void* logs_q, const void* m_p, const void* logs_p,
                      const int32_t* lens, float* out2, void* stream);
int evt_masked_kl_bwd(const evt_kl_params* p, const void* z_p, const void* logs_q, const void* m_p, const void* logs_p,
                      const int32_t* lens, const float* dloss, const float* count, void* dz_p, void* dlogs_q, void* dm_p,
                      void* dlogs_p, void* stream);

typedef struct evt_adamw_seg { int64_t begin, end; float lr; float weight_decay; } evt_adamw_seg;
int evt_adamw_flat(float* param, const float* grad, float* exp_avg, float* exp_avg_sq, int64_t n,
                   const evt_adamw_seg* segs, int32_t nseg, float beta1, float beta2, float eps, int32_t step,
                   float grad_scale, void* stream);
int evt_adamw_flat_dev(float* param, const float* grad, float* exp_avg, float* exp_avg_sq, int64_t n,
                       const evt_adamw_seg* segs, int32_t nseg, float beta1, float beta2, float eps,
                       int32_t* step_counter, float grad_scale, void* stream);
int evt_adamw_flat_dev_range(float* param, const float* grad, float* exp_avg, float* exp_avg_sq, int64_t lo, int64_t hi,
                             const evt_adamw_seg* segs, int32_t nseg, float beta1, float beta2, float eps,
                             int32_t* step_counter, int32_t bump, float grad_scale, void* stream);
int evt_mpd_fold(int32_t src0_dtype, const void* src0, int32_t n0, int32_t src1_dtype, const void* src1, int32_t n1, int32_t T,
                 const int32_t* periods, int32_t nper, void* const* outs, int32_t out_dtype, void* stream);
int evt_mpd_unfold(int32_t grad_dtype, const void* const* douts, const int32_t* periods, int32_t nper, int32_t b0, int32_t n,
                   int32_t T, int32_t dsrc_dtype, void* dsrc, void* stream);

int evt_sumsq(const float* x, int64_t n, float* out, void* stream);

int evt_scaler_unscale(float* grad, int64_t n, const float* scale, float* found_inf, void* stream);
int evt_adamw_flat_dev_guarded(float* param, const float* grad, float* exp_avg, float* exp_avg_sq, int64_t n,
                               const evt_adamw_seg* segs, int32_t nseg, float beta1, float beta2, float eps,
                               int32_t* step_counter, float grad_scale, const float* skip, void* stream);
int evt_scaler_update(float* scale, int32_t* growth_tracker, float* const* found_inf, int32_t nflags, float growth_factor,
                      float backoff_factor, int32_t growth_interval, void* stream);

typedef struct evt_gemm_params {
  int32_t dtype;
  int32_t M, N, K;
  int32_t relu;
} evt_gemm_params;
int evt_gemm_bf16_layout(const evt_gemm_params* g, evt_wlayout* out);
int evt_gemm_bf16_fwd(const evt_gemm_params* g, const void* x, const void* w_reg, const void* w_alt, const float* bias,
                      void* y, void* stream);
int evt_gemm_bf16_bwd_data(const evt_gemm_params* g, const void* dy, const void* w_reg, const void* w_alt, void* dx,
                           void* stream);
int evt_gemm_bf16_bwd_weight(const evt_gemm_params* g, const void* x, const void* dy, float* dw, float* dbias,
                             void* stream);

typedef struct evt_gemm_epilogue {
  float dropout_p;
  uint32_t site;
  const uint32_t* seed_dev;
  const void* gate;
  float gate_pos;
  uint32_t pad_;
  const void* add;
} evt_gemm_epilogue;
int32_t evt_gemm_bf16_fused_supported(const evt_gemm_params* g, int32_t backward_data);
int evt_gemm_bf16_fwd_ex(const evt_gemm_params* g, const void* x, const void* w_reg, const void* w_alt, const float* bias,
                         const evt_gemm_epilogue* epi, void* y, void* stream);
int evt_gemm_bf16_bwd_data_ex(const evt_gemm_params* g, const void* dy, const void* w_reg, const void* w_alt,
                              const evt_gemm_epilogue* epi, void* dx, void* stream);

typedef struct evt_attn_params {
  int32_t dtype, B, L, H, D;
  int32_t x_len;
  int64_t q_stride_b, q_stride_l, q_stride_h;
  int64_t o_stride_b, o_stride_l, o_stride_h;
  float dropout_p;
  uint32_t seed;
} evt_attn_params;
int evt_attn_prefixlm_fwd(const evt_attn_params* p, const void* q, const void* k, const void* v,
                          const int32_t* x_lens, const int32_t* y_lens, void* o, float* lse, void* stream);
int evt_attn_prefixlm_bwd(const evt_attn_params* p, const void* q, const void* k, const void* v, const void* o,
                          const void* d_o, const float* lse, const int32_t* x_lens, const int32_t* y_lens,
                          void* dq, void* dk, void* dv, float* delta_ws, void* stream);

int evt_add_layernorm_fwd(int32_t dtype, const void* x, const void* r, const float* gamma, const float* beta,
                          void* y, float* mean, float* rstd, int64_t rows, int32_t C, float eps, void* stream);
int evt_add_layernorm_bwd(int32_t dtype, const void* x, const void* r, const float* gamma, const void* dy,
                          const float* mean, const float* rstd, void* dxr, float* dgamma, float* dbeta,
                          int64_t rows, int32_t C, void* stream);

int evt_counter_inc(uint32_t* counter, uint32_t inc, void* stream);

int evt_res_dropout_ln_fwd(int32_t dtype, const void* x, const void* y, const float* gamma, const float* beta,
                           const int32_t* lens, int32_t rows_per_seq, float p, const uint32_t* seed_dev, uint32_t site,
                           void* out, float* mean, float* rstd, int64_t rows, int32_t C, float eps, void* stream);
int evt_res_dropout_ln_bwd(int32_t dtype, const void* x, const void* y, const float* gamma, const void* dout,
                           const float* mean, const float* rstd, const int32_t* lens, int32_t rows_per_seq, float p,
                           const uint32_t* seed_dev, uint32_t site, void* dx, void* dy, float* dgamma, float* dbeta,
                           int64_t rows, int32_t C, void* stream);

int evt_relu_dropout_fwd(int32_t dtype, const void* x, float p, const uint32_t* seed_dev, uint32_t site,
                         const int32_t* lens, int32_t rows_per_seq, int32_t C, void* y, int64_t n, void* stream);
int evt_relu_dropout_bwd(int32_t dtype, const void* x, const void* dy, float p, const uint32_t* seed_dev, uint32_t site,
                         const int32_t* lens, int32_t rows_per_seq, int32_t C, void* dx, int64_t n, void* stream);

int evt_wn_residual_fwd(int32_t dtype, const void* x, const void* rs, const void* acc, const int32_t* lens,
                        int32_t rows_per_seq, void* x_out, void* acc_out, int64_t rows, int32_t H, int32_t last,
                        void* stream);
int evt_mish_dropout_fwd(int32_t dtype, int32_t wide_dtype, const void* x, float p, const uint32_t* seed_dev, uint32_t site,
                         void* y, int64_t n, void* stream);
int evt_mish_dropout_bwd(int32_t dtype, int32_t wide_dtype, const void* x, const void* dy, float p, const uint32_t* seed_dev,
                         uint32_t site, void* dx, int64_t n, void* stream);
int evt_glu_dropout_res_fwd(int32_t dtype, int32_t wide_dtype, const void* h, const void* res, float p,
                            const uint32_t* seed_dev, uint32_t site, void* y, int64_t rows, int32_t C, void* stream);
int evt_glu_dropout_res_bwd(int32_t dtype, int32_t wide_dtype, const void* h, const void* dy, float p,
                            const uint32_t* seed_dev, uint32_t site, void* dh, int64_t rows, int32_t C, void* stream);
#define EVT_MEAN_ROWS_CHUNK 64
int evt_mish_rows_fwd(int32_t dtype, int32_t wide_dtype, const void* x, const int32_t* lens, int32_t nseq, int32_t L,
                      int32_t C, void* y, void* stream);
int evt_glu_res_rows_fwd(int32_t dtype, int32_t wide_dtype, const void* h, const void* res, const int32_t* lens,
                         int32_t nseq, int32_t L, int32_t C, void* y, void* stream);
int evt_mean_rows(int32_t dtype, const void* x, const int32_t* lens, int32_t nseq, int32_t L, int32_t C, float* out,
                  void* stream);
int evt_reparam_fwd(int32_t dtype, const void* stats, const float* eps, const int32_t* lens, int32_t rows_per_seq,
                    int64_t rows, int32_t C, float* z, float* m, float* logs, void* stream);
int evt_reparam_bwd(int32_t dtype, const float* dz, const float* dm, const float* dlogs, const float* eps, const float* logs,
                    const int32_t* lens, int32_t rows_per_seq, int64_t rows, int32_t C, void* dstats, void* stream);
int evt_coupling_flip_fwd(int32_t dtype, const float* x, const void* stats, const int32_t* lens, int32_t rows_per_seq,
                          int64_t rows, int32_t h, float* y, void* x0n, void* stream);
int evt_coupling_flip_bwd(int32_t dtype, const float* dy, const void* dx0n, const int32_t* lens, int32_t rows_per_seq,
                          int64_t rows, int32_t h, float* dx, void* dstats, void* stream);
int evt_wn_residual_bwd(int32_t dtype, const void* dx_out, const void* dacc_out, const int32_t* lens,
                        int32_t rows_per_seq, void* dx, void* drs, int64_t rows, int32_t H, int32_t last, void* stream);

typedef struct evt_mha_params {
  int32_t dtype;
  int32_t B, H, D;
  int32_t Tq, Tk;
  int32_t window;
  int32_t n_heads_rel;
  int64_t ldq, ldk, ldo;
  float scale;
  float dropout_p;
  uint32_t site;
  uint32_t pad_;
  const uint32_t* seed_dev;
} evt_mha_params;
int evt_mha_fwd(const evt_mha_params* p, const void* q, const void* k, const void* v, const float* emb_k,
                const float* emb_v, const int32_t* lens_q, const int32_t* lens_k, void* out, float* lse, void* stream);
int evt_mha_bwd(const evt_mha_params* p, const void* q, const void* k, const void* v, const void* o, const void* d_o,
                const float* lse, const float* emb_k, const float* emb_v, const int32_t* lens_q, const int32_t* lens_k,
                void* dq, void* dk, void* dv, float* demb_k, float* demb_v, float* delta_ws, void* stream);

int evt_ce_sum_fwd_bwd(int32_t dtype, const void* logits, const int64_t* targets, void* dlogits, float* loss,
                       int32_t* hits, int64_t rows, int32_t V, int32_t topk, int64_t ignore_index, float dloss,
                       void* stream);
int evt_ce_rows_fwd_bwd(int32_t dtype, const void* logits, const int64_t* targets, void* dlogits, float* row_loss,
                        int32_t* hits, int64_t rows, int32_t V, int32_t topk, int64_t ignore_index, void* stream);
int evt_ce_sum_fwd_bwd_ld(int32_t dtype, const void* logits, const int64_t* targets, void* dlogits, float* loss,
                          int32_t* hits, int64_t rows, int32_t V, int64_t ld, int32_t topk, int64_t ignore_index,
                          float dloss, void* stream);
int evt_ce_rows_fwd_bwd_ld(int32_t dtype, const void* logits, const int64_t* targets, void* dlogits, float* row_loss,
                           int32_t* hits, int64_t rows, int32_t V, int64_t ld, int32_t topk, int64_t ignore_index,
                           void* stream);

#define EVT_DEC_POS 0
#define EVT_DEC_IDX 1
#define EVT_DEC_YCOUNT 2
#define EVT_DEC_YLEN 3
#define EVT_DEC_SEED 4
int evt_dec_gemv(int32_t wdtype, const void* W, const float* bias, const float* a, const float* r, const float* ln_g,
                 const float* ln_b, float ln_eps, float* x_out, float* y, int32_t B, int32_t N, int32_t K, int32_t relu,
                 void* stream);
int evt_dec_gemm_rows(int32_t wdtype, const void* W, const float* bias, const float* a, const float* r,
                      const float* ln_g, const float* ln_b, float ln_eps, float* x_out, float* y, int32_t B, int32_t N,
                      int32_t K, int32_t relu, void* stream);
int evt_dec_attn(int32_t cdtype, const float* qkv, void* kcache, void* vcache, const int32_t* ctr, float* out, int32_t B,
                 int32_t H, int32_t D, int32_t Lmax, const int32_t* x_lens, int32_t x_len, void* stream);
int evt_dec_qkv_attn(int32_t dtype, const void* Wqkv, const float* bqkv, const float* a, const float* r,
                     const float* ln_g, const float* ln_b, float ln_eps, float* x_out, void* kcache, void* vcache,
                     const int32_t* ctr, float* out, int32_t B, int32_t H, int32_t D, int32_t Lmax, const int32_t* x_lens,
                     int32_t x_len, void* stream);
typedef struct evt_sample_params {
  int32_t V, eos, top_k, no_eos_steps, ymax;
  float top_p, temperature, repetition_penalty;
  uint32_t seed;
  int32_t noise_rows;
} evt_sample_params;
int evt_dec_sample(const evt_sample_params* p, const float* logits, int64_t* y, const int32_t* ctr, const float* noise,
                   int32_t* stop_idx, float* probs_out, int32_t B, void* stream);
int evt_dec_sample_rows(const evt_sample_params* p, const float* logits, int64_t* y, const int32_t* ctr,
                        const float* noise, int32_t* stop_idx, float* probs_out, const int32_t* row_seed, int32_t B,
                        void* stream);
int evt_dec_sample_embed(const evt_sample_params* p, const float* logits, int64_t* y, int32_t* ctr, const float* noise,
                         int32_t* stop_idx, const float* emb, const float* pe, const float* alpha, float x_scale, float* x,
                         int32_t E, int32_t npos, int32_t dpos, void* stream);
int evt_dec_embed(const float* emb, const float* pe, const float* alpha, float x_scale, const int64_t* y,
                  const int32_t* ctr, float* x, int32_t B, int32_t E, int32_t ymax, int32_t npos, void* stream);
int evt_dec_advance(int32_t* ctr, int32_t dpos, void* stream);

#define EVT_ROW_WORDS 8
#define EVT_ROW_POS 0
#define EVT_ROW_IDX 1
#define EVT_ROW_YCOUNT 2
#define EVT_ROW_YLEN 3
#define EVT_ROW_LIMIT 4
#define EVT_ROW_STATUS 5
#define EVT_ROW_NOISE 6
#define EVT_ROW_NFORCE 7
#define EVT_ROW_SPARE EVT_ROW_NFORCE
#define EVT_ROW_IDLE 0
#define EVT_ROW_RUNNING 1
#define EVT_ROW_STOP_EOS 2
#define EVT_ROW_STOP_LIMIT 3
int evt_dec_attn_rows(int32_t cdtype, const float* qkv, void* kcache, void* vcache, const int32_t* rstate, float* out,
                      int32_t B, int32_t H, int32_t D, int32_t Lmax, const int32_t* x_lens, int32_t x_len, void* stream);
int evt_dec_sample_embed_rows(const evt_sample_params* p, const float* logits, int64_t* y, int32_t* rstate,
                              const float* noise, int32_t* stop_idx, float* probs_out, const int32_t* row_seed,
                              const int32_t* row_mask, const float* emb, const float* pe, const float* alpha,
                              float x_scale, float* x, int32_t B, int32_t E, int32_t npos, int32_t dpos, void* stream);
typedef struct evt_row_sample { int32_t top_k; float top_p, temperature, repetition_penalty; } evt_row_sample;
int evt_dec_sample_embed_rows_p(const evt_sample_params* p, const evt_row_sample* row_sample, const float* logits,
                                int64_t* y, int32_t* rstate, const float* noise, int32_t* stop_idx, float* probs_out,
                                const int32_t* row_seed, const int32_t* row_mask, const float* emb, const float* pe,
                                const float* alpha, float x_scale, float* x, int32_t B, int32_t E, int32_t npos,
                                int32_t dpos, void* stream);
int evt_dec_sample_embed_rows_lp(const evt_sample_params* p, const evt_row_sample* row_sample, const float* logits,
                                 int64_t* y, int32_t* rstate, const float* noise, int32_t* stop_idx, float* probs_out,
                                 const int32_t* row_seed, const int32_t* row_mask, const float* emb, const float* pe,
                                 const float* alpha, float x_scale, float* x, float* row_logp, int32_t B, int32_t E,
                                 int32_t npos, int32_t dpos, void* stream);
int evt_dec_sample_embed_rows_f(const evt_sample_params* p, const evt_row_sample* row_sample, const float* logits,
                                int64_t* y, int32_t* rstate, const float* noise, int32_t* stop_idx, float* probs_out,
                                const int32_t* row_seed, const int32_t* row_mask, const float* emb, const float* pe,
                                const float* alpha, float x_scale, float* x, float* row_logp, int32_t B, int32_t E,
                                int32_t npos, int32_t dpos, void* stream);

typedef struct evt_sa_chunk { int64_t begin, end; int32_t tensor; int32_t pad_; } evt_sa_chunk;
typedef struct evt_scaled_adam_hp {
  float lr, beta1, beta2, eps, scalar_lr_scale, scalar_max;
  int32_t step, pad_;
} evt_scaled_adam_hp;
int evt_scaled_adam_stats(const float* param, const float* grad, const evt_sa_chunk* chunks, int32_t nchunks,
                          float* stats, void* stream);
int evt_scaled_adam_apply(float* param, const float* grad, float* delta, float* exp_avg_sq, const evt_sa_chunk* chunks,
                          int32_t nchunks, const float* coef, const evt_scaled_adam_hp* hp, void* stream);

int evt_gelu_rows_fwd(int32_t dtype, const void* x, const float* bias, void* out, int64_t nseq, int32_t t_in, int32_t t_out,
                      int32_t C, void* stream);
int evt_channel_norm_gelu_fwd(int32_t dtype, const void* x, const float* gamma, const float* beta, float eps, void* out,
                              int32_t nseq, int32_t T, int32_t C, int32_t apply_gelu, void* stream);

#define EVT_HUBERT_FRONT_CHUNK 64
int64_t evt_hubert_front_ws_floats(int32_t nseq, int32_t N);
int evt_hubert_front_rows(int32_t dtype, const float* wav, const int32_t* lens, int32_t nseq, int32_t N, const float* w,
                          const float* gamma, const float* beta, float eps, void* out, float* ws, int64_t ws_floats,
                          void* stream);

int evt_clip_rescale_rows(const float* x, const int32_t* lens, int32_t nseq, int32_t N, float* f, int16_t* q, float* peak,
                          void* stream);

int evt_phone_expand_rows(int32_t dtype, const void* h, int32_t B, int32_t T, int32_t C, const int32_t* src,
                          const int32_t* item_off, int32_t n_items, int32_t total, int32_t out_dtype, void* out,
                          void* stream);

int evt_bert_embed_ln_rows(int32_t dtype, const int32_t* ids, const int32_t* tt, const int32_t* lens, int32_t B, int32_t T,
                           const float* word, int32_t vocab, const float* pos, int32_t max_pos, const float* type,
                           int32_t types, const float* gamma, const float* beta, float eps, int32_t C, void* out,
                           void* stream);

int evt_rms_frames_rows(const float* x, int64_t x_len, const int64_t* off, const int64_t* len, int32_t nrec, int32_t win,
                        int32_t hop, float* rms, const int64_t* frame_off, int64_t total_frames, void* stream);

int evt_span_peak_rows(const float* x, int64_t x_len, const int64_t* src_off, const int64_t* n, int32_t nspan, int64_t max_n,
                       float* peak, void* stream);

int evt_slice_pack_rows(const float* x, int64_t x_len, const int64_t* src_off, const int64_t* n, const int64_t* dst_off,
                        const float* peak, float c1, float c2, int32_t nspan, int64_t max_n, int16_t* out, int64_t out_len,
                        void* stream);

#define EVT_SEMANTIC_TILE 32
#define EVT_SEMANTIC_MAX_D 1152
int evt_semantic_codes_rows(int32_t dtype, const void* hs, const int32_t* frames, const int32_t* frames_host,
                            const int64_t* offsets, int32_t B, int32_t Tmax, int32_t D, int32_t K, const float* proj_image,
                            const float* bias, const float* embed, const float* ee, int64_t* codes, int64_t total,
                            void* stream);

#pragma GCC visibility pop
#ifdef __cplusplus
}
#endif
#endif
```

Baseline: 3575 audio-s/s.

## Fuse WN stack entry and exit 1x1 projections into first and last layer kernels

Folds the pre-projection (entry) into the first WN layer's launch and the post/proj projection (exit) into the last layer's launch, in both forward and backward kernels. Each fused kernel computes the extra 1x1 conv from shared-memory tiles already resident, which removes separate projection launches and the global round-trips of the hidden tensor. The Python side routes PosteriorEncoder and coupling layers through the fused paths when supported and falls back otherwise. This adds template variants and more registers and shared memory per block, and the entry path recomputes the projection over halo rows.

```diff
diff --git a/easevoice_trainer_amd/csrc/wn_layer.hip b/easevoice_trainer_amd/csrc/wn_layer.hip
--- a/easevoice_trainer_amd/csrc/wn_layer.hip
+++ b/easevoice_trainer_amd/csrc/wn_layer.hip
@@ -19,6 +19,13 @@
   h16_t* acts;
   h16_t* x_out;
   h16_t* acc_out;
+  const h16_t* w_x;
+  const float* b_x;
+  h16_t* stats;
+  const h16_t* x0;
+  const h16_t* w_e;
+  const float* b_e;
+  h16_t* h_out;
   int nseq, L, tps;
 };
 
@@ -34,7 +41,7 @@
   o[2] = h2f_lo(v[1]); o[3] = h2f_hi(v[1]);
 }
 
-template <int H, int K, int NT, int R, bool LAST>
+template <int H, int K, int NT, int R, bool LAST, int CX, int CE>
 __global__ __launch_bounds__(256, 1) void wn_layer_fwd(WNP p) {
   constexpr int PITCH = H * 2;
   constexpr int SPR = H / 8;
@@ -46,10 +53,19 @@
   constexpr int NKA = NCH * K, NKB = NCH;
   constexpr int MA = 2 * MT;
   constexpr int MB = LAST ? MT : 2 * MT;
+  constexpr int XT = CX / 16;
+  constexpr int MX = (XT + 3) / 4;
+  constexpr int NKX = NCH;
+  constexpr int NKE = CE / 32;
+  constexpr int NTE = (XROWS + 15) / 16;
+  static_assert(CE == 0 || (!LAST && CE % 32 == 0 && CE <= H), "entry projection: not on a last layer, rows within the x pitch");
   static_assert(H % 64 == 0 && SPR % 8 == 0, "rows of whole 128-byte groups, M-tiles divisible by the four waves");
+  static_assert(CX == 0 || (LAST && CX % 16 == 0 && XT % MX == 0 && MX <= MA && NKX <= R - 1 && P <= XROWS),
+                "exit projection: last layer, waves with MX tiles or none, all of its fragments in one ring fill");
   extern __shared__ __attribute__((aligned(1024))) unsigned char smem[];
   unsigned char* xs = smem;
   unsigned char* acl = smem + ((XROWS + 7) & ~7) * PITCH;
+  unsigned char* x0s = acl + P * PITCH;
   const int tid = threadIdx.x, lane = tid & 63, wm = __builtin_amdgcn_readfirstlane(tid >> 6);
   const int n = lane & 15, g = lane >> 4;
   const int seq = blockIdx.x / p.tps;
@@ -68,23 +84,46 @@
   };
   using CA = std::integral_constant<int, MA>;
   using CB = std::integral_constant<int, MB>;
-
-  constexpr int NP = XROWS * SPR;
+  const bool xwave = CX > 0 && wm * MX < XT;
+  auto issue_x = [&](const int ks, const int s) {
+#pragma unroll
+    for (int i = 0; i < MX; ++i)
+      fa[s][i] = *reinterpret_cast<const u32x4*>(p.w_x + ((long)((wm * MX + i) * NKX + ks) * 64 + lane) * 8);
+  };
+
+  constexpr int SPRX = (CE > 0 ? CE : H) / 8;
+  constexpr int NP = XROWS * SPRX;
   constexpr int PER = (NP + 255) / 256;
+  u32x4 fe[NKE > 0 ? NKE : 1][MT];
+  if constexpr (CE > 0) {
+#pragma unroll
+    for (int ks = 0; ks < NKE; ++ks)
+#pragma unroll
+      for (int i = 0; i < MT; ++i)
+        fe[ks][i] = *reinterpret_cast<const u32x4*>(p.w_e + ((long)((wm * MT + i) * NKE + ks) * 64 + lane) * 8);
+  }
+  f32x4 bE[MT];
+#pragma unroll
+  for (int i = 0; i < MT; ++i)
+    bE[i] = (CE > 0 && p.b_e) ? *reinterpret_cast<const f32x4*>(p.b_e + (wm * MT + i) * 16 + g * 4) : f32x4{0.f, 0.f, 0.f, 0.f};
   uint4 xv[PER];
 #pragma unroll
   for (int u = 0; u < PER; ++u) {
     const int idx = u * 256 + tid;
-    const int r = idx / SPR, sl = idx - r * SPR;
+    const int r = idx / SPRX, sl = idx - r * SPRX;
     const int pos = q0 - HALO + r;
-    xv[u] = (idx < NP && pos >= 0 && pos < p.L) ? *reinterpret_cast<const uint4*>(p.x + (sbase + pos) * H + sl * 8)
-                                                : make_uint4(0, 0, 0, 0);
+    const h16_t* src = CE > 0 ? p.x0 + (sbase + pos) * CE + sl * 8 : p.x + (sbase + pos) * H + sl * 8;
+    xv[u] = (idx < NP && pos >= 0 && pos < p.L) ? *reinterpret_cast<const uint4*>(src) : make_uint4(0, 0, 0, 0);
   }
 #pragma unroll
   for (int s = 0; s < R - 1 && s < NKA; ++s) issue_a(p.w_in, NKA, s, s, CA{});
   float bA0[MT][4], bA1[MT][4], bB0[MT][4], bB1[MT][4];
   u32x2 gA0[MT], gA1[MT], accp[MT][NT];
   const int len = p.lens ? p.lens[seq] : p.L;
+  f32x4 bX[MX > 0 ? MX : 1];
+#pragma unroll
+  for (int i = 0; i < MX; ++i)
+    bX[i] = (xwave && p.b_x) ? *reinterpret_cast<const f32x4*>(p.b_x + (wm * MX + i) * 16 + g * 4) : f32x4{0.f, 0.f, 0.f, 0.f};
 #pragma unroll
   for (int i = 0; i < MT; ++i) {
     const int h = (wm * MT + i) * 16 + g * 4;
@@ -110,12 +149,49 @@
   for (int u = 0; u < PER; ++u) {
     const int idx = u * 256 + tid;
     if (idx >= NP) continue;
-    const int r = idx / SPR, sl = idx - r * SPR;
-    *reinterpret_cast<uint4*>(xs + r * PITCH + wslot(r, sl) * 16) = xv[u];
+    const int r = idx / SPRX, sl = idx - r * SPRX;
+    *reinterpret_cast<uint4*>((CE > 0 ? x0s : xs) + r * PITCH + wslot(r, sl) * 16) = xv[u];
   }
   __syncthreads();
 
-  auto conv = [&](auto& acc, const h16_t* w, auto nk_c, auto taps_c, auto cnt, const unsigned char* rows) {
+  if constexpr (CE > 0) {
+    f32x4 acc[MT][NTE];
+#pragma unroll
+    for (int i = 0; i < MT; ++i)
+#pragma unroll
+      for (int j = 0; j < NTE; ++j) acc[i][j] = f32x4{0.f, 0.f, 0.f, 0.f};
+#pragma unroll
+    for (int ks = 0; ks < NKE; ++ks) {
+      const unsigned char* b0 = x0s + n * PITCH + wslot(n, ks * 4 + g) * 16;
+#pragma unroll
+      for (int j = 0; j < NTE; ++j) {
+        const u32x4 fb = *reinterpret_cast<const u32x4*>(b0 + j * 16 * PITCH);
+#pragma unroll
+        for (int i = 0; i < MT; ++i) acc[i][j] = EVT_MFMA_16x16x32(as_h8(fe[ks][i]), as_h8(fb), acc[i][j], 0, 0, 0);
+      }
+    }
+#pragma unroll
+    for (int i = 0; i < MT; ++i) {
+      const int h = (wm * MT + i) * 16 + g * 4;
+      const f32x4 be = bE[i];
+#pragma unroll
+      for (int j = 0; j < NTE; ++j) {
+        const int m = j * 16 + n;
+        const int pos = q0 - HALO + m;
+        if (m >= XROWS) continue;
+        const bool live = pos >= 0 && pos < p.L && pos < len;
+        h16_t o4[4];
+#pragma unroll
+        for (int r = 0; r < 4; ++r) o4[r] = f2h(live ? acc[i][j][r] + be[r] : 0.f);
+        *reinterpret_cast<uint2*>(xs + m * PITCH + wslot(m, h >> 3) * 16 + (h & 7) * 2) = *reinterpret_cast<uint2*>(o4);
+        if (m >= HALO && m < HALO + P && pos < p.L)
+          *reinterpret_cast<uint2*>(p.h_out + (sbase + pos) * H + h) = *reinterpret_cast<uint2*>(o4);
+      }
+    }
+    __syncthreads();
+  }
+
+  auto conv = [&](auto& acc, auto issue, auto nk_c, auto taps_c, auto cnt, const unsigned char* rows) {
     constexpr int NK = decltype(nk_c)::value, TAPS = decltype(taps_c)::value, CNT = decltype(cnt)::value;
     u32x4 fb[NT];
     auto b_addr = [&](const int ks) {
@@ -133,7 +209,7 @@
 #pragma unroll
     for (int ks = 0; ks < NK; ++ks) {
       const int s = ks % R;
-      if (ks + R - 1 < NK) issue_a(w, NK, ks + R - 1, (ks + R - 1) % R, cnt);
+      if (ks + R - 1 < NK) issue(ks + R - 1, (ks + R - 1) % R);
 #pragma unroll
       for (int i = 0; i < CNT; ++i) tie(fa[s][i]);
       const unsigned char* nb = b_addr(ks + 1 < NK ? ks + 1 : ks);
@@ -154,7 +230,8 @@
     for (int i = 0; i < MA; ++i)
 #pragma unroll
       for (int j = 0; j < NT; ++j) acc[i][j] = f32x4{0.f, 0.f, 0.f, 0.f};
-    conv(acc, p.w_in, std::integral_constant<int, NKA>{}, std::integral_constant<int, K>{}, CA{}, xs);
+    conv(acc, [&](const int ks, const int s) { issue_a(p.w_in, NKA, ks, s, CA{}); }, std::integral_constant<int, NKA>{},
+         std::integral_constant<int, K>{}, CA{}, xs);
 #pragma unroll
     for (int s = 0; s < R - 1 && s < NKB; ++s) issue_a(p.w_rs, NKB, s, s, CB{});
 #pragma unroll
@@ -193,7 +270,14 @@
     for (int i = 0; i < MB; ++i)
 #pragma unroll
       for (int j = 0; j < NT; ++j) acc[i][j] = f32x4{0.f, 0.f, 0.f, 0.f};
-    conv(acc, p.w_rs, std::integral_constant<int, NKB>{}, std::integral_constant<int, 1>{}, CB{}, acl);
+    conv(acc, [&](const int ks, const int s) { issue_a(p.w_rs, NKB, ks, s, CB{}); }, std::integral_constant<int, NKB>{},
+         std::integral_constant<int, 1>{}, CB{}, acl);
+    if constexpr (CX > 0) {
+      if (xwave) {
+#pragma unroll
+        for (int s = 0; s < NKX; ++s) issue_x(s, s);
+      }
+    }
 #pragma unroll
     for (int i = 0; i < MT; ++i) {
       const int h = (wm * MT + i) * 16 + g * 4;
@@ -201,8 +285,8 @@
       for (int j = 0; j < NT; ++j) {
         const int m = j * 16 + n;
         const int pos = q0 + m;
-        if (pos >= p.L) continue;
-        const bool live = pos < len;
+        if (CX == 0 && pos >= p.L) continue;
+        const bool live = pos < len && pos < p.L;
         float ap[4];
         unpack4(accp[i][j], ap);
         h16_t o1[4], o2[4];
@@ -211,6 +295,10 @@
           for (int r = 0; r < 4; ++r) {
             const float rs = h2f(f2h(acc[i][j][r] + bB0[i][r]));
             o2[r] = f2h(live ? ap[r] + rs : 0.f);
+          }
+          if constexpr (CX > 0) {
+            *reinterpret_cast<uint2*>(xs + m * PITCH + wslot(m, h >> 3) * 16 + (h & 7) * 2) = *reinterpret_cast<uint2*>(o2);
+            if (pos >= p.L) continue;
           }
         } else {
           float xo[4];
@@ -226,6 +314,32 @@
           *reinterpret_cast<uint2*>(p.x_out + (sbase + pos) * H + h) = *reinterpret_cast<uint2*>(o1);
         }
         *reinterpret_cast<uint2*>(p.acc_out + (sbase + pos) * H + h) = *reinterpret_cast<uint2*>(o2);
+      }
+    }
+  }
+
+  if constexpr (CX > 0) {
+    __syncthreads();
+    if (xwave) {
+      f32x4 acc[MX][NT];
+#pragma unroll
+      for (int i = 0; i < MX; ++i)
+#pragma unroll
+        for (int j = 0; j < NT; ++j) acc[i][j] = f32x4{0.f, 0.f, 0.f, 0.f};
+      conv(acc, issue_x, std::integral_constant<int, NKX>{}, std::integral_constant<int, 1>{},
+           std::integral_constant<int, MX>{}, xs);
+#pragma unroll
+      for (int i = 0; i < MX; ++i) {
+        const int c = (wm * MX + i) * 16 + g * 4;
+#pragma unroll
+        for (int j = 0; j < NT; ++j) {
+          const int pos = q0 + j * 16 + n;
+          if (pos >= p.L) continue;
+          h16_t o4[4];
+#pragma unroll
+          for (int r = 0; r < 4; ++r) o4[r] = f2h(acc[i][j][r] + bX[i][r]);
+          *reinterpret_cast<uint2*>(p.stats + (sbase + pos) * CX + c) = *reinterpret_cast<uint2*>(o4);
+        }
       }
     }
   }
@@ -243,6 +357,10 @@
   h16_t* dx_in;
   h16_t* dx;
   float* dg;
+  const h16_t* dstats;
+  const h16_t* w_x;
+  const h16_t* w_e;
+  h16_t* dx0;
   int nseq, L, tps;
 };
 
@@ -256,7 +374,7 @@
   return v;
 }
 
-template <int H, int K, int NT, int R, bool LAST>
+template <int H, int K, int NT, int R, bool LAST, int CX, int CE>
 __global__ __launch_bounds__(256, 1) void wn_layer_bwd(WNB p) {
   constexpr int PB = H * 4;
   constexpr int SPRB = H / 4;
@@ -267,10 +385,18 @@
   constexpr int ROWS = P + 2 * HALO;
   constexpr int CIN1 = LAST ? H : 2 * H;
   constexpr int NK1 = CIN1 / 32, NK2 = (2 * H / 32) * K;
+  constexpr int NKX = CX / 32;
   static_assert(2 * HALO <= 16, "one extra position tile covers the halo");
+  static_assert(CX == 0 || (LAST && CX % 32 == 0 && CX <= 2 * H), "exit projection: last layer, rows that fit a dx_in row");
+  constexpr int ET = CE / 16;
+  constexpr int ME = (ET + 3) / 4;
+  constexpr int NKE = H / 32;
+  static_assert(CE == 0 || (!LAST && CE % 16 == 0 && ET % ME == 0 && ME <= MT && NKE <= R - 1),
+                "entry projection: not on a last layer, waves with ME tiles or none, all of its fragments in one ring fill");
   extern __shared__ __attribute__((aligned(1024))) unsigned char smem[];
   unsigned char* ds = smem;
   unsigned char* es = smem + 16 * NT1 * PB;
+  unsigned char* hs = smem + 2 * 16 * NT1 * PB;
   const int tid = threadIdx.x, lane = tid & 63, wm = __builtin_amdgcn_readfirstlane(tid >> 6);
   const int n = lane & 15, g = lane >> 4;
   const int seq = blockIdx.x / p.tps;
@@ -285,7 +411,15 @@
       fa[s][i] = *reinterpret_cast<const u32x4*>(w + ((long)((wm * MT + i) * nk + ks) * 64 + lane) * 8);
   };
 
-  constexpr int SPR1 = CIN1 / 8;
+  using CM = std::integral_constant<int, MT>;
+  const bool ewave = CE > 0 && wm * ME < ET;
+  auto issue_e = [&](const int ks, const int s) {
+#pragma unroll
+    for (int i = 0; i < ME; ++i)
+      fa[s][i] = *reinterpret_cast<const u32x4*>(p.w_e + ((long)((wm * ME + i) * NKE + ks) * 64 + lane) * 8);
+  };
+
+  constexpr int SPR1 = (CX > 0 ? CX : CIN1) / 8;
   constexpr int NP = ROWS * SPR1;
   constexpr int PER = (NP + 255) / 256;
   uint4 dv[PER];
@@ -296,7 +430,9 @@
     const int pos = q0 - HALO + r;
     uint4 v = make_uint4(0, 0, 0, 0);
     if (idx < NP && pos >= 0 && pos < p.L) {
-      if (LAST) {
+      if (CX > 0) {
+        v = *reinterpret_cast<const uint4*>(p.dstats + (sbase + pos) * CX + sl * 8);
+      } else if (LAST) {
         if (pos < len) v = *reinterpret_cast<const uint4*>(p.dacc + (sbase + pos) * H + sl * 8);
       } else if (sl < H / 8) {
         if (p.dx_next && pos < len) v = *reinterpret_cast<const uint4*>(p.dx_next + (sbase + pos) * H + sl * 8);
@@ -306,8 +442,13 @@
     }
     dv[u] = v;
   }
-#pragma unroll
-  for (int s = 0; s < R - 1 && s < NK1; ++s) issue_a(p.w_rs, NK1, s, s);
+  if constexpr (CX > 0) {
+#pragma unroll
+    for (int s = 0; s < R - 1 && s < NKX; ++s) issue_a(p.w_x, NKX, s, s);
+  } else {
+#pragma unroll
+    for (int s = 0; s < R - 1 && s < NK1; ++s) issue_a(p.w_rs, NK1, s, s);
+  }
   u32x2 xa[MT][NT1], xb[MT][NT1], ga[MT], gb[MT];
 #pragma unroll
   for (int i = 0; i < MT; ++i) {
@@ -331,15 +472,20 @@
     const int idx = u * 256 + tid;
     if (idx >= NP) continue;
     const int r = idx / SPR1, sl = idx - r * SPR1;
-    *reinterpret_cast<uint4*>(ds + r * PB + wslot2(r, sl) * 16) = dv[u];
-    const int pos = q0 - HALO + r;
-    if (r >= HALO && r < HALO + P && pos < p.L)
-      *reinterpret_cast<uint4*>(p.drs + (sbase + pos) * CIN1 + sl * 8) = dv[u];
+    if constexpr (CX > 0) {
+      *reinterpret_cast<uint4*>(es + r * PB + wslot2(r, sl) * 16) = dv[u];
+    } else {
+      *reinterpret_cast<uint4*>(ds + r * PB + wslot2(r, sl) * 16) = dv[u];
+      const int pos = q0 - HALO + r;
+      if (r >= HALO && r < HALO + P && pos < p.L)
+        *reinterpret_cast<uint4*>(p.drs + (sbase + pos) * CIN1 + sl * 8) = dv[u];
+    }
   }
   __syncthreads();
 
-  auto conv = [&](auto& acc, const h16_t* w, auto nk_c, auto taps_c, auto nt_c, const unsigned char* rows) {
+  auto conv = [&](auto& acc, auto issue, auto nk_c, auto taps_c, auto nt_c, auto cnt, const unsigned char* rows) {
     constexpr int NK = decltype(nk_c)::value, TAPS = decltype(taps_c)::value, NTC = decltype(nt_c)::value;
+    constexpr int CNT = decltype(cnt)::value;
     u32x4 fb[NTC];
     auto b_addr = [&](const int ks) {
       const int ch = ks / TAPS, tap = ks - ch * TAPS;
@@ -354,28 +500,59 @@
 #pragma unroll
     for (int ks = 0; ks < NK; ++ks) {
       const int s = ks % R;
-      if (ks + R - 1 < NK) issue_a(w, NK, ks + R - 1, (ks + R - 1) % R);
-#pragma unroll
-      for (int i = 0; i < MT; ++i) tie(fa[s][i]);
+      if (ks + R - 1 < NK) issue(ks + R - 1, (ks + R - 1) % R);
+#pragma unroll
+      for (int i = 0; i < CNT; ++i) tie(fa[s][i]);
       const unsigned char* nb = b_addr(ks + 1 < NK ? ks + 1 : ks);
 #pragma unroll
       for (int j = 0; j < NTC; ++j) {
         tie(fb[j]);
 #pragma unroll
-        for (int i = 0; i < MT; ++i)
+        for (int i = 0; i < CNT; ++i)
           acc[i][j] = EVT_MFMA_16x16x32(as_h8(fa[s][i]), as_h8(fb[j]), acc[i][j], 0, 0, 0);
         fb[j] = *reinterpret_cast<const u32x4*>(nb + j * 16 * PB);
       }
     }
   };
 
+  if constexpr (CX > 0) {
+    f32x4 acc[MT][NT1];
+#pragma unroll
+    for (int i = 0; i < MT; ++i)
+#pragma unroll
+      for (int j = 0; j < NT1; ++j) acc[i][j] = f32x4{0.f, 0.f, 0.f, 0.f};
+    conv(acc, [&](const int ks, const int s) { issue_a(p.w_x, NKX, ks, s); }, std::integral_constant<int, NKX>{},
+         std::integral_constant<int, 1>{}, std::integral_constant<int, NT1>{}, CM{}, es);
+#pragma unroll
+    for (int s = 0; s < R - 1 && s < NK1; ++s) issue_a(p.w_rs, NK1, s, s);
+#pragma unroll
+    for (int i = 0; i < MT; ++i) {
+      const int h = (wm * MT + i) * 16 + g * 4;
+#pragma unroll
+      for (int j = 0; j < NT1; ++j) {
+        const int m = j * 16 + n;
+        const int pos = q0 - HALO + m;
+        const bool in = m < ROWS && pos >= 0 && pos < p.L;
+        const bool live = in && pos < len;
+        h16_t o4[4];
+#pragma unroll
+        for (int r = 0; r < 4; ++r) o4[r] = f2h(live ? acc[i][j][r] : 0.f);
+        *reinterpret_cast<uint2*>(ds + m * PB + wslot2(m, h >> 3) * 16 + (h & 7) * 2) = *reinterpret_cast<uint2*>(o4);
+        if (in && m >= HALO && m < HALO + P)
+          *reinterpret_cast<uint2*>(p.drs + (sbase + pos) * H + h) = *reinterpret_cast<uint2*>(o4);
+      }
+    }
+    __syncthreads();
+  }
+
   {
     f32x4 acc[MT][NT1];
 #pragma unroll
     for (int i = 0; i < MT; ++i)
 #pragma unroll
       for (int j = 0; j < NT1; ++j) acc[i][j] = f32x4{0.f, 0.f, 0.f, 0.f};
-    conv(acc, p.w_rs, std::integral_constant<int, NK1>{}, std::integral_constant<int, 1>{}, std::integral_constant<int, NT1>{}, ds);
+    conv(acc, [&](const int ks, const int s) { issue_a(p.w_rs, NK1, ks, s); }, std::integral_constant<int, NK1>{},
+         std::integral_constant<int, 1>{}, std::integral_constant<int, NT1>{}, CM{}, ds);
 #pragma unroll
     for (int s = 0; s < R - 1 && s < NK2; ++s) issue_a(p.w_in, NK2, s, s);
 #pragma unroll
@@ -432,7 +609,14 @@
     for (int i = 0; i < MT; ++i)
 #pragma unroll
       for (int j = 0; j < NT; ++j) acc[i][j] = f32x4{0.f, 0.f, 0.f, 0.f};
-    conv(acc, p.w_in, std::integral_constant<int, NK2>{}, std::integral_constant<int, K>{}, std::integral_constant<int, NT>{}, es);
+    conv(acc, [&](const int ks, const int s) { issue_a(p.w_in, NK2, ks, s); }, std::integral_constant<int, NK2>{},
+         std::integral_constant<int, K>{}, std::integral_constant<int, NT>{}, CM{}, es);
+    if constexpr (CE > 0) {
+      if (ewave) {
+#pragma unroll
+        for (int s = 0; s < NKE; ++s) issue_e(s, s);
+      }
+    }
 #pragma unroll
     for (int i = 0; i < MT; ++i) {
       const int h = (wm * MT + i) * 16 + g * 4;
@@ -440,16 +624,50 @@
       for (int j = 0; j < NT; ++j) {
         const int m = j * 16 + n;
         const int pos = q0 + m;
-        if (pos >= p.L) continue;
+        if (CE == 0 && pos >= p.L) continue;
         float dr[4] = {0.f, 0.f, 0.f, 0.f};
         if (!LAST) {
           const int r0 = HALO + m;
           unpack4(*reinterpret_cast<const u32x2*>(ds + r0 * PB + wslot2(r0, h >> 3) * 16 + (h & 7) * 2), dr);
         }
         h16_t o4[4];
-#pragma unroll
-        for (int r = 0; r < 4; ++r) o4[r] = f2h(acc[i][j][r] + dr[r]);
+        if constexpr (CE > 0) {
+          const bool live = pos < len && pos < p.L;
+#pragma unroll
+          for (int r = 0; r < 4; ++r) o4[r] = f2h(live ? acc[i][j][r] + dr[r] : 0.f);
+          *reinterpret_cast<uint2*>(hs + m * PB + wslot2(m, h >> 3) * 16 + (h & 7) * 2) = *reinterpret_cast<uint2*>(o4);
+          if (pos >= p.L) continue;
+        } else {
+#pragma unroll
+          for (int r = 0; r < 4; ++r) o4[r] = f2h(acc[i][j][r] + dr[r]);
+        }
         *reinterpret_cast<uint2*>(p.dx + (sbase + pos) * H + h) = *reinterpret_cast<uint2*>(o4);
+      }
+    }
+  }
+
+  if constexpr (CE > 0) {
+    __syncthreads();
+    if (ewave) {
+      f32x4 acc[ME][NT];
+#pragma unroll
+      for (int i = 0; i < ME; ++i)
+#pragma unroll
+        for (int j = 0; j < NT; ++j) acc[i][j] = f32x4{0.f, 0.f, 0.f, 0.f};
+      conv(acc, issue_e, std::integral_constant<int, NKE>{}, std::integral_constant<int, 1>{}, std::integral_constant<int, NT>{},
+           std::integral_constant<int, ME>{}, hs);
+#pragma unroll
+      for (int i = 0; i < ME; ++i) {
+        const int c = (wm * ME + i) * 16 + g * 4;
+#pragma unroll
+        for (int j = 0; j < NT; ++j) {
+          const int pos = q0 + j * 16 + n;
+          if (pos >= p.L) continue;
+          h16_t o4[4];
+#pragma unroll
+          for (int r = 0; r < 4; ++r) o4[r] = f2h(acc[i][j][r]);
+          *reinterpret_cast<uint2*>(p.dx0 + (sbase + pos) * CE + c) = *reinterpret_cast<uint2*>(o4);
+        }
       }
     }
   }
@@ -469,30 +687,34 @@
   }
 }
 
-template <int NT, int R, bool LAST>
+template <int NT, int R, bool LAST, int CX = 0, int CE = 0>
 int launch(WNP p, hipStream_t st) {
   constexpr int H = 192, K = 5, P = 16 * NT;
   p.tps = (p.L + P - 1) / P;
-  const size_t lds = (size_t)(((P + K - 1 + 7) & ~7) + P) * H * 2;
-  evt_set_last_tag("wn_layer_fwd<%s, %d, k%d, nt %d, ring %d%s>", EVT_HALF_NAME, H, K, NT, R, LAST ? ", last" : "");
-  hipLaunchKernelGGL((wn_layer_fwd<H, K, NT, R, LAST>), dim3(p.nseq * p.tps), dim3(256), lds, st, p);
+  const size_t lds = (size_t)(((P + K - 1 + 7) & ~7) + P + (CE > 0 ? (P + K - 1 + 15) / 16 * 16 : 0)) * H * 2;
+  if (CE > 0) evt_set_last_tag("wn_layer_fwd<%s, %d, k%d, nt %d, ring %d, entry %d>", EVT_HALF_NAME, H, K, NT, R, CE);
+  else if (CX > 0) evt_set_last_tag("wn_layer_fwd<%s, %d, k%d, nt %d, ring %d, last, exit %d>", EVT_HALF_NAME, H, K, NT, R, CX);
+  else evt_set_last_tag("wn_layer_fwd<%s, %d, k%d, nt %d, ring %d%s>", EVT_HALF_NAME, H, K, NT, R, LAST ? ", last" : "");
+  hipLaunchKernelGGL((wn_layer_fwd<H, K, NT, R, LAST, CX, CE>), dim3(p.nseq * p.tps), dim3(256), lds, st, p);
   return evt_check_launch();
 }
 
-template <int NT, int R, bool LAST>
+template <int NT, int R, bool LAST, int CX = 0, int CE = 0>
 int launch_b(WNB p, hipStream_t st) {
   constexpr int H = 192, K = 5, P = 16 * NT;
   p.tps = (p.L + P - 1) / P;
-  const size_t lds = (size_t)2 * 16 * (NT + 1) * H * 4;
+  const size_t lds = (size_t)(2 * 16 * (NT + 1) + (CE > 0 ? P : 0)) * H * 4;
   static bool attr = false;
   if (!attr && lds > 64 * 1024) {
-    if (hipFuncSetAttribute(reinterpret_cast<const void*>(&wn_layer_bwd<H, K, NT, R, LAST>),
+    if (hipFuncSetAttribute(reinterpret_cast<const void*>(&wn_layer_bwd<H, K, NT, R, LAST, CX, CE>),
                             hipFuncAttributeMaxDynamicSharedMemorySize, 160 * 1024) != hipSuccess)
       return EVT_ELAUNCH;
     attr = true;
   }
-  evt_set_last_tag("wn_layer_bwd<%s, %d, k%d, nt %d, ring %d%s>", EVT_HALF_NAME, H, K, NT, R, LAST ? ", last" : "");
-  hipLaunchKernelGGL((wn_layer_bwd<H, K, NT, R, LAST>), dim3(p.nseq * p.tps), dim3(256), lds, st, p);
+  if (CE > 0) evt_set_last_tag("wn_layer_bwd<%s, %d, k%d, nt %d, ring %d, entry %d>", EVT_HALF_NAME, H, K, NT, R, CE);
+  else if (CX > 0) evt_set_last_tag("wn_layer_bwd<%s, %d, k%d, nt %d, ring %d, last, exit %d>", EVT_HALF_NAME, H, K, NT, R, CX);
+  else evt_set_last_tag("wn_layer_bwd<%s, %d, k%d, nt %d, ring %d%s>", EVT_HALF_NAME, H, K, NT, R, LAST ? ", last" : "");
+  hipLaunchKernelGGL((wn_layer_bwd<H, K, NT, R, LAST, CX, CE>), dim3(p.nseq * p.tps), dim3(256), lds, st, p);
   return evt_check_launch();
 }
 
@@ -540,4 +762,78 @@
   return last ? launch_b<1, 8, true>(p, st) : launch_b<1, 8, false>(p, st);
 }
 
-}
+int32_t evt_wn_layer_exit_supported(int32_t dtype, int32_t H, int32_t k, int32_t dil, int32_t cout) {
+  return (evt_wn_layer_supported(dtype, H, k, dil) && (cout == 96 || cout == 384)) ? 1 : 0;
+}
+
+int evt_wn_layer_fwd_exit(int32_t dtype, const void* x, const void* w_in_frag, const float* b_in, const void* w_rs_frag,
+                          const float* b_rs, const void* g, const void* acc_in, const int32_t* lens, void* x_in, void* acts,
+                          void* acc_out, const void* w_exit_frag, const float* b_exit, void* stats, int32_t nseq, int32_t L,
+                          int32_t H, int32_t k, int32_t cout, void* stream) {
+  if (!evt_wn_layer_exit_supported(dtype, H, k, 1, cout)) return EVT_ENOTSUP;
+  if (!x || !w_in_frag || !w_rs_frag || !x_in || !acts || !acc_out || !w_exit_frag || !stats || nseq <= 0 || L <= 0)
+    return EVT_EINVAL;
+  WNP p{};
+  p.x = (const h16_t*)x; p.w_in = (const h16_t*)w_in_frag; p.w_rs = (const h16_t*)w_rs_frag; p.b_in = b_in; p.b_rs = b_rs;
+  p.g = (const h16_t*)g; p.acc_in = (const h16_t*)acc_in; p.lens = lens;
+  p.x_in = (h16_t*)x_in; p.acts = (h16_t*)acts; p.acc_out = (h16_t*)acc_out;
+  p.w_x = (const h16_t*)w_exit_frag; p.b_x = b_exit; p.stats = (h16_t*)stats;
+  p.nseq = nseq; p.L = L;
+  hipStream_t st = (hipStream_t)stream;
+  return cout == 96 ? launch<1, 8, true, 96>(p, st) : launch<1, 8, true, 384>(p, st);
+}
+
+int evt_wn_layer_bwd_data_exit(int32_t dtype, const void* dstats, const void* w_exit_alt_frag, const void* x_in, const void* g,
+                               const void* w_rs_alt_frag, const void* w_in_alt_frag, const int32_t* lens, void* drs,
+                               void* dx_in, void* dx, float* dg, int32_t nseq, int32_t L, int32_t H, int32_t k, int32_t cout,
+                               void* stream) {
+  if (!evt_wn_layer_exit_supported(dtype, H, k, 1, cout)) return EVT_ENOTSUP;
+  if (!dstats || !w_exit_alt_frag || !x_in || !w_rs_alt_frag || !w_in_alt_frag || !drs || !dx_in || !dx || nseq <= 0 || L <= 0)
+    return EVT_EINVAL;
+  WNB p{};
+  p.dstats = (const h16_t*)dstats; p.w_x = (const h16_t*)w_exit_alt_frag; p.x_in = (const h16_t*)x_in; p.g = (const h16_t*)g;
+  p.w_rs = (const h16_t*)w_rs_alt_frag; p.w_in = (const h16_t*)w_in_alt_frag; p.lens = lens;
+  p.drs = (h16_t*)drs; p.dx_in = (h16_t*)dx_in; p.dx = (h16_t*)dx; p.dg = dg;
+  p.nseq = nseq; p.L = L;
+  hipStream_t st = (hipStream_t)stream;
+  return cout == 96 ? launch_b<1, 8, true, 96>(p, st) : launch_b<1, 8, true, 384>(p, st);
+}
+
+int32_t evt_wn_layer_entry_supported(int32_t dtype, int32_t H, int32_t k, int32_t dil, int32_t cin, int32_t n_layers) {
+  return (evt_wn_layer_supported(dtype, H, k, dil) && cin == 96 && n_layers >= 2) ? 1 : 0;
+}
+
+int evt_wn_layer_fwd_entry(int32_t dtype, const void* x0, const void* w_entry_frag, const float* b_entry, int32_t cin,
+                           const void* w_in_frag, const float* b_in, const void* w_rs_frag, const float* b_rs, const void* g,
+                           const int32_t* lens, void* h, void* x_in, void* acts, void* x_out, void* acc_out, int32_t nseq,
+                           int32_t L, int32_t H, int32_t k, void* stream) {
+  if (!evt_wn_layer_entry_supported(dtype, H, k, 1, cin, 2)) return EVT_ENOTSUP;
+  if (!x0 || !w_entry_frag || !w_in_frag || !w_rs_frag || !h || !x_in || !acts || !x_out || !acc_out || nseq <= 0 || L <= 0)
+    return EVT_EINVAL;
+  WNP p{};
+  p.x0 = (const h16_t*)x0; p.w_e = (const h16_t*)w_entry_frag; p.b_e = b_entry; p.h_out = (h16_t*)h;
+  p.w_in = (const h16_t*)w_in_frag; p.w_rs = (const h16_t*)w_rs_frag; p.b_in = b_in; p.b_rs = b_rs;
+  p.g = (const h16_t*)g; p.lens = lens;
+  p.x_in = (h16_t*)x_in; p.acts = (h16_t*)acts; p.x_out = (h16_t*)x_out; p.acc_out = (h16_t*)acc_out;
+  p.nseq = nseq; p.L = L;
+  return launch<1, 8, false, 0, 96>(p, (hipStream_t)stream);
+}
+
+int evt_wn_layer_bwd_data_entry(int32_t dtype, const void* dx_next, const void* dacc, const void* x_in, const void* g,
+                                const void* w_rs_alt_frag, const void* w_in_alt_frag, const int32_t* lens, void* drs,
+                                void* dx_in, void* dh, float* dg, const void* w_entry_alt_frag, void* dx0, int32_t nseq,
+                                int32_t L, int32_t H, int32_t k, int32_t cin, void* stream) {
+  if (!evt_wn_layer_entry_supported(dtype, H, k, 1, cin, 2)) return EVT_ENOTSUP;
+  if (!dacc || !x_in || !w_rs_alt_frag || !w_in_alt_frag || !drs || !dx_in || !dh || !w_entry_alt_frag || !dx0 || nseq <= 0 ||
+      L <= 0)
+    return EVT_EINVAL;
+  WNB p{};
+  p.dx_next = (const h16_t*)dx_next; p.dacc = (const h16_t*)dacc; p.x_in = (const h16_t*)x_in; p.g = (const h16_t*)g;
+  p.w_rs = (const h16_t*)w_rs_alt_frag; p.w_in = (const h16_t*)w_in_alt_frag; p.lens = lens;
+  p.drs = (h16_t*)drs; p.dx_in = (h16_t*)dx_in; p.dx = (h16_t*)dh; p.dg = dg;
+  p.w_e = (const h16_t*)w_entry_alt_frag; p.dx0 = (h16_t*)dx0;
+  p.nseq = nseq; p.L = L;
+  return launch_b<1, 8, false, 0, 96>(p, (hipStream_t)stream);
+}
+
+}
diff --git a/easevoice_trainer_amd/hip/wn.py b/easevoice_trainer_amd/hip/wn.py
--- a/easevoice_trainer_amd/hip/wn.py
+++ b/easevoice_trainer_amd/hip/wn.py
@@ -6,17 +6,21 @@
 
 class WNStackFn(torch.autograd.Function):
     @staticmethod
-    def forward(ctx, x, g_lbh, lens, anchor, in_slots, rs_slots, hidden):
+    def forward(ctx, x, g_lbh, lens, anchor, in_slots, rs_slots, hidden, exit_slot=None, entry_slot=None):
         n_layers, H = len(in_slots), hidden
         B, T, _ = x.shape
-        if not x.is_contiguous() or x.size(2) != H or (g_lbh is not None and not g_lbh.is_contiguous()):
+        win = H if entry_slot is None else entry_slot.module.cin
+        if not x.is_contiguous() or x.size(2) != win or (g_lbh is not None and not g_lbh.is_contiguous()):
             raise L.EvtError("WN stack: contiguous [B, T, H] input and [n_layers, B, 2H] conditioning expected")
         dt = L.dt_of(x)
         rows = B * T
         saved = []
-        out = None
+        out = x0 = None
         fused = FUSED_FORWARD and _layer_fused(dt, H, in_slots, rs_slots)
+        if (exit_slot is not None or entry_slot is not None) and not fused:
+            raise L.EvtError("WN stack: entry / exit projections go with the one-launch layer forward (wn_stack decides)")
         frag_in, frag_rs = _frag_images(in_slots, rs_slots) if fused else (None, None)
+        stats = None
         for i in range(n_layers):
             last = i == n_layers - 1
             if fused:
@@ -26,6 +30,42 @@
                 acc_out = torch.empty((B, T, H), dtype=x.dtype, device=x.device)
                 x_out = None if last else torch.empty_like(acc_out)
                 e0 = HC._t0()
+                if i == 0 and entry_slot is not None:
+                    men = entry_slot.module
+                    h = torch.empty((B, T, H), dtype=x.dtype, device=x.device)
+                    L.check(L.lib().evt_wn_layer_fwd_entry(dt, L.ptr(x), L.ptr(entry_slot.bank.frag(entry_slot, "reg")),
+                                                           L.ptr(men.bias.data if men.bias is not None else None), men.cin,
+                                                           L.ptr(frag_in[i]),
+                                                           L.ptr(mi.bias.data if mi.bias is not None else None),
+                                                           L.ptr(frag_rs[i]),
+                                                           L.ptr(mr.bias.data if mr.bias is not None else None),
+                                                           L.ptr(g_lbh[i] if g_lbh is not None else None), L.ptr(lens),
+                                                           L.ptr(h), L.ptr(x_in), L.ptr(acts), L.ptr(x_out), L.ptr(acc_out),
+                                                           B, T, H, mi.k, L.stream_ptr()), "evt_wn_layer_fwd_entry")
+                    x0, x = x, h
+                    if e0 is not None:
+                        _t1_layer(e0, mi, mr, x, mx=men)
+                    saved += [x, x_in, acts]
+                    x, out = x_out, acc_out
+                    continue
+                if last and exit_slot is not None:
+                    me = exit_slot.module
+                    stats = torch.empty((B, T, me.cout), dtype=x.dtype, device=x.device)
+                    L.check(L.lib().evt_wn_layer_fwd_exit(dt, L.ptr(x), L.ptr(frag_in[i]),
+                                                          L.ptr(mi.bias.data if mi.bias is not None else None),
+                                                          L.ptr(frag_rs[i]),
+                                                          L.ptr(mr.bias.data if mr.bias is not None else None),
+                                                          L.ptr(g_lbh[i] if g_lbh is not None else None), L.ptr(out),
+                                                          L.ptr(lens), L.ptr(x_in), L.ptr(acts), L.ptr(acc_out),
+                                                          L.ptr(exit_slot.bank.frag(exit_slot, "reg")),
+                                                          L.ptr(me.bias.data if me.bias is not None else None),
+                                                          L.ptr(stats), B, T, H, mi.k, me.cout, L.stream_ptr()),
+                            "evt_wn_layer_fwd_exit")
+                    if e0 is not None:
+                        _t1_layer(e0, mi, mr, x, mx=me)
+                    saved += [x, x_in, acts]
+                    x, out = x_out, acc_out
+                    continue
                 L.check(L.lib().evt_wn_layer_fwd(dt, L.ptr(x), L.ptr(frag_in[i]),
                                                  L.ptr(mi.bias.data if mi.bias is not None else None), L.ptr(frag_rs[i]),
                                                  L.ptr(mr.bias.data if mr.bias is not None else None),
@@ -49,14 +89,18 @@
                                                 L.stream_ptr()), "evt_wn_residual_fwd")
             saved += [x, x_in, acts]
             x, out = x_out, acc_out
+        if entry_slot is not None:
+            saved.append(x0)
+        if exit_slot is not None:
+            saved.append(out)
         ctx.save_for_backward(lens, g_lbh, *saved)
-        ctx.cfg = (in_slots, rs_slots, H, B, T)
-        return out
+        ctx.cfg = (in_slots, rs_slots, H, B, T, exit_slot, entry_slot)
+        return out if exit_slot is None else stats
 
     @staticmethod
     def backward(ctx, dout):
         lens, g_lbh, *saved = ctx.saved_tensors
-        in_slots, rs_slots, H, B, T = ctx.cfg
+        in_slots, rs_slots, H, B, T, exit_slot, entry_slot = ctx.cfg
         n_layers = len(in_slots)
         dtype, dev = dout.dtype, dout.device
         dt = L.dt_code(dtype)
@@ -65,6 +109,17 @@
         dx_next = None
         dg32 = torch.zeros((n_layers, B, 2 * H), dtype=torch.float32, device=dev) if g_lbh is not None else None
         fused = FUSED_BACKWARD and _layer_fused(dt, H, in_slots, rs_slots)
+        dstats = None
+        if exit_slot is not None:
+            out = saved.pop()
+            dstats, dacc = dacc, None
+            if exit_slot.bank.weight_grads:
+                HC._bwd_weight(exit_slot, out, dstats, None, B, T, 1.0, L.ACT_NONE, 1.0)
+            if not (fused and FUSED_EXIT):
+                dacc = HC._bwd_data(exit_slot, dstats, None, out, None, B, T, 1.0, L.ACT_NONE, 1.0)
+                dstats = None
+        x0 = saved.pop() if entry_slot is not None else None
+        dx0 = None
         group = [] if (GROUP_WGRADS and HC.TRACE is None) else None
 
         def wgrad(*args):
@@ -86,14 +141,35 @@
                 dx_in = torch.empty((B, T, 2 * H), dtype=dtype, device=dev)
                 dx = torch.empty((B, T, H), dtype=dtype, device=dev)
                 e0 = HC._t0()
-                L.check(L.lib().evt_wn_layer_bwd_data(dt, L.ptr(dx_next), L.ptr(dacc), L.ptr(x_in),
-                                                      L.ptr(g_lbh[i] if g_lbh is not None else None),
-                                                      L.ptr(sr.bank.frag(sr, "alt")), L.ptr(si.bank.frag(si, "alt")),
-                                                      L.ptr(lens), L.ptr(drs), L.ptr(dx_in), L.ptr(dx),
-                                                      L.ptr(dg32[i] if dg32 is not None else None), B, T, H, si.module.k,
-                                                      int(last), L.stream_ptr()), "evt_wn_layer_bwd_data")
+                entry = i == 0 and entry_slot is not None and FUSED_ENTRY
+                if entry:
+                    dx0 = torch.empty((B, T, entry_slot.module.cin), dtype=dtype, device=dev)
+                    L.check(L.lib().evt_wn_layer_bwd_data_entry(dt, L.ptr(dx_next), L.ptr(dacc), L.ptr(x_in),
+                                                                L.ptr(g_lbh[i] if g_lbh is not None else None),
+                                                                L.ptr(sr.bank.frag(sr, "alt")), L.ptr(si.bank.frag(si, "alt")),
+                                                                L.ptr(lens), L.ptr(drs), L.ptr(dx_in), L.ptr(dx),
+                                                                L.ptr(dg32[i] if dg32 is not None else None),
+                                                                L.ptr(entry_slot.bank.frag(entry_slot, "alt")), L.ptr(dx0),
+                                                                B, T, H, si.module.k, entry_slot.module.cin, L.stream_ptr()),
+                            "evt_wn_layer_bwd_data_entry")
+                elif last and dstats is not None:
+                    L.check(L.lib().evt_wn_layer_bwd_data_exit(dt, L.ptr(dstats), L.ptr(exit_slot.bank.frag(exit_slot, "alt")),
+                                                               L.ptr(x_in), L.ptr(g_lbh[i] if g_lbh is not None else None),
+                                                               L.ptr(sr.bank.frag(sr, "alt")), L.ptr(si.bank.frag(si, "alt")),
+                                                               L.ptr(lens), L.ptr(drs), L.ptr(dx_in), L.ptr(dx),
+                                                               L.ptr(dg32[i] if dg32 is not None else None), B, T, H,
+                                                               si.module.k, exit_slot.module.cout, L.stream_ptr()),
+                            "evt_wn_layer_bwd_data_exit")
+                else:
+                    L.check(L.lib().evt_wn_layer_bwd_data(dt, L.ptr(dx_next), L.ptr(dacc), L.ptr(x_in),
+                                                          L.ptr(g_lbh[i] if g_lbh is not None else None),
+                                                          L.ptr(sr.bank.frag(sr, "alt")), L.ptr(si.bank.frag(si, "alt")),
+                                                          L.ptr(lens), L.ptr(drs), L.ptr(dx_in), L.ptr(dx),
+                                                          L.ptr(dg32[i] if dg32 is not None else None), B, T, H, si.module.k,
+                                                          int(last), L.stream_ptr()), "evt_wn_layer_bwd_data")
                 if e0 is not None:
-                    _t1_layer(e0, si.module, sr.module, x, "bwd_data")
+                    _t1_layer(e0, si.module, sr.module, x, "bwd_data",
+                              mx=entry_slot.module if entry else exit_slot.module if (last and dstats is not None) else None)
                 if last:
                     dacc = drs
                 if sr.bank.weight_grads:
@@ -119,16 +195,27 @@
             s = in_slots[i]
             if s.bank.weight_grads:
                 wgrad(s, x, dx_in, None, B, T, 1.0, L.ACT_NONE, 1.0)
-            need_dx = i > 0 or ctx.needs_input_grad[0]
+            need_dx = i > 0 or ctx.needs_input_grad[0] or entry_slot is not None
             dx_next = HC._bwd_data(s, dx_in, None, x, dx_res, B, T, 1.0, L.ACT_NONE, 1.0) if need_dx else None
         if group:
             HC._bwd_weight_group(group)
+        if entry_slot is not None:
+            dh = dx_next
+            if dx0 is None:
+                dh = dx_next * (torch.arange(T, device=dev)[None, :] < lens[:, None]).unsqueeze(-1).to(dtype)
+                if ctx.needs_input_grad[0]:
+                    dx0 = HC._bwd_data(entry_slot, dh, None, x0, None, B, T, 1.0, L.ACT_NONE, 1.0)
+            if entry_slot.bank.weight_grads:
+                HC._bwd_weight(entry_slot, x0, dh, None, B, T, 1.0, L.ACT_NONE, 1.0)
+            dx_next = dx0
         dg = dg32.to(g_lbh.dtype) if (dg32 is not None and ctx.needs_input_grad[1]) else None
-        return dx_next, dg, None, None, None, None, None
+        return dx_next, dg, None, None, None, None, None, None, None
 
 
 FUSED_FORWARD = True
 FUSED_BACKWARD = True
+FUSED_ENTRY = True
+FUSED_EXIT = True
 GROUP_WGRADS = True
 GROUP_LAYERS = 2
 
@@ -157,12 +244,34 @@
     return True
 
 
+def _exit_fused(dt, H, in_slots, rs_slots, exit_slot):
+    if not (FUSED_FORWARD and FUSED_EXIT and _layer_fused(dt, H, in_slots, rs_slots)):
+        return False
+    me, mi = exit_slot.module, in_slots[0].module
+    if exit_slot.bank is not in_slots[0].bank or exit_slot.packed_member:
+        return False
+    if (me.cin, me.k, me.stride, me.groups, me.pad, me.dil, me.transposed) != (H, 1, 1, 1, 0, 1, False):
+        return False
+    return bool(L.lib().evt_wn_layer_exit_supported(dt, H, mi.k, mi.dil, me.cout))
+
+
+def _entry_fused(dt, H, in_slots, rs_slots, entry_slot):
+    if not (FUSED_FORWARD and FUSED_ENTRY and _layer_fused(dt, H, in_slots, rs_slots)):
+        return False
+    me, mi = entry_slot.module, in_slots[0].module
+    if entry_slot.bank is not in_slots[0].bank or entry_slot.packed_member or getattr(me, "src_d1", me.cin) != me.cin:
+        return False
+    if (me.cout, me.k, me.stride, me.groups, me.pad, me.dil, me.transposed) != (H, 1, 1, 1, 0, 1, False):
+        return False
+    return bool(L.lib().evt_wn_layer_entry_supported(dt, H, mi.k, mi.dil, me.cin, len(in_slots)))
+
+
 def _frag_images(in_slots, rs_slots):
     bank = in_slots[0].bank
     return [bank.frag(s, "reg") for s in in_slots], [bank.frag(s, "reg") for s in rs_slots]
 
 
-def _t1_layer(e0, mi, mr, x, kind="fwd"):
+def _t1_layer(e0, mi, mr, x, kind="fwd", mx=None):
     e0, rf = e0
     e1 = torch.cuda.Event(enable_timing=True)
     e1.record()
@@ -170,14 +279,38 @@
         rf.__exit__(None, None, None)
     n, ln, h = x.shape
     macs = n * ln * (mi.cin * mi.cout * mi.k + mr.cin * mr.cout)
-    HC.TRACE.append((L.lib().evt_last_kernel_tag().decode(), kind, 2 * macs,
-                     (7 * x.numel() + mi.v.numel() + mr.v.numel()) * 2, e0, e1,
-                     f"WN layer {h}>{mi.cout}>{mr.cout} k{mi.k} n{n} L{ln}", mi))
-
-
-def wn_stack(x, g_lbh, lens, in_layers, rs_layers, hidden):
+    elems = 7 * x.numel() + mi.v.numel() + mr.v.numel()
+    shape = f"WN layer {h}>{mi.cout}>{mr.cout} k{mi.k} n{n} L{ln}"
+    if mx is not None:
+        macs += n * ln * mx.cin * mx.cout
+        elems += n * ln * mx.cout + mx.v.numel()
+        shape += f" +exit {mx.cout}"
+    HC.TRACE.append((L.lib().evt_last_kernel_tag().decode(), kind, 2 * macs, elems * 2, e0, e1, shape, mi))
+
+
+def entry_fused(x, in_layers, rs_layers, hidden, entry_layer):
+    in_slots = tuple(m._slot for m in in_layers)
+    rs_slots = tuple(m._slot for m in rs_layers)
+    es = entry_layer._slot
+    if es is None or any(s is None for s in in_slots + rs_slots) or not x.is_cuda or x.dtype != es.bank.dtype:
+        return False
+    return _entry_fused(L.dt_of(x), int(hidden), in_slots, rs_slots, es)
+
+
+def wn_stack(x, g_lbh, lens, in_layers, rs_layers, hidden, exit_layer=None, entry_layer=None):
     in_slots = tuple(m._slot for m in in_layers)
     rs_slots = tuple(m._slot for m in rs_layers)
     if any(s is None for s in in_slots + rs_slots):
         raise L.EvtError("WN stack before WeightBank.attach(); there is no eager fallback")
-    return WNStackFn.apply(x, g_lbh, lens, in_slots[0].bank.anchor, in_slots, rs_slots, int(hidden))
+    anchor = in_slots[0].bank.anchor
+    es = None
+    if entry_layer is not None:
+        es = entry_layer._slot
+        if es is None or not _entry_fused(L.dt_of(x), int(hidden), in_slots, rs_slots, es):
+            raise L.EvtError("WN stack: this entry projection is not served by the first layer's launch (ask entry_fused first)")
+    if exit_layer is not None:
+        xs = exit_layer._slot
+        if xs is not None and _exit_fused(L.dt_of(x), int(hidden), in_slots, rs_slots, xs):
+            return WNStackFn.apply(x, g_lbh, lens, anchor, in_slots, rs_slots, int(hidden), xs, es)
+        return exit_layer(WNStackFn.apply(x, g_lbh, lens, anchor, in_slots, rs_slots, int(hidden), None, es))
+    return WNStackFn.apply(x, g_lbh, lens, anchor, in_slots, rs_slots, int(hidden), None, es)
diff --git a/easevoice_trainer_amd/module/models.py b/easevoice_trainer_amd/module/models.py
--- a/easevoice_trainer_amd/module/models.py
+++ b/easevoice_trainer_amd/module/models.py
@@ -11,7 +11,7 @@
 from ..hip.conv import Add3ScaleFn, EvtConv1d, GatedActFn, mask_tail, res_stage, res_unit, resample_rows
 from ..hip.enc import new_site, rel_self_attention, unbind_rows, wn_residual, wn_residual_last
 from ..hip.frontend import RvqEncoder, ncl_to_nlc
-from ..hip.wn import wn_stack
+from ..hip.wn import entry_fused, wn_stack
 from . import commons
 from .attentions import Encoder, MultiHeadAttention, PointwiseEvtConv, linear_rows, pointwise
 
@@ -51,8 +51,14 @@
             rs = 2 * hidden_channels if i < n_layers - 1 else hidden_channels
             self.res_skip_layers.append(EvtConv1d(hidden_channels, rs, 1, weight_norm=True))
 
-    def forward(self, x, x_mask, g=None, lens=None):
+    def entry_fused(self, x, entry_layer):
+        return (not (self.training and self.drop.p > 0)
+                and entry_fused(x, self.in_layers, self.res_skip_layers, self.hidden_channels, entry_layer))
+
+    def forward(self, x, x_mask, g=None, lens=None, exit_layer=None, entry_layer=None):
         H = self.hidden_channels
+        if entry_layer is not None and not self.entry_fused(x, entry_layer):
+            raise L.EvtError("WN.forward: this entry projection is not served inside the stack (ask entry_fused first)")
         if lens is None:
             lens = x_mask.sum(dim=(1, 2)).to(torch.int32)
         x = x.contiguous()
@@ -60,7 +66,7 @@
             g_lbh = None
             if g is not None:
                 g_lbh = self.cond_layer(g).to(x.dtype).view(g.size(0), self.n_layers, 2 * H).transpose(0, 1).contiguous()
-            return wn_stack(x, g_lbh, lens, self.in_layers, self.res_skip_layers, H)
+            return wn_stack(x, g_lbh, lens, self.in_layers, self.res_skip_layers, H, exit_layer, entry_layer)
         gs = None
         if g is not None:
             g = self.cond_layer(g).to(x.dtype)
@@ -74,7 +80,7 @@
                 x, output = wn_residual(x, rs, output, lens)
             else:
                 output = wn_residual_last(rs, output, lens)
-        return output
+        return output if exit_layer is None else exit_layer(output)
 
 
 class PosteriorEncoder(nn.Module, _ComputeDtype):
@@ -91,14 +97,14 @@
         if g is not None:
             g = g.detach()
         h = (self.pre(x) * x_mask).to(self.cd).contiguous()
-        h = self.enc(h, x_mask, g=g, lens=lens)
         if h.is_cuda and lens is not None:
             from ..hip.enc import reparam
 
-            stats = self.proj(h)
+            stats = self.enc(h, x_mask, g=g, lens=lens, exit_layer=self.proj)
             if eps is None:
                 eps = torch.randn((stats.size(0), stats.size(1), self.out_channels), dtype=torch.float32, device=h.device)
             return reparam(stats, eps, lens)
+        h = self.enc(h, x_mask, g=g, lens=lens)
         stats = self.proj(h) * x_mask
         m, logs = torch.split(stats.float(), self.out_channels, dim=-1)
         if eps is None:
@@ -141,9 +147,14 @@
 
         if x0c is None:
             x0c = x[..., :self.half_channels]
-        h = (self.pre(x0c) * mask_cd).contiguous()
-        h = self.enc(h, x_mask, g=g, lens=lens)
-        return coupling_flip(x, self.post(h), lens, want_next)
+        if x0c.dtype != self.cd or not x0c.is_contiguous():
+            x0c = x0c.to(self.cd).contiguous()
+        if self.enc.entry_fused(x0c, self.pre):
+            stats = self.enc(x0c, x_mask, g=g, lens=lens, exit_layer=self.post, entry_layer=self.pre)
+        else:
+            h = (self.pre(x0c) * mask_cd).contiguous()
+            stats = self.enc(h, x_mask, g=g, lens=lens, exit_layer=self.post)
+        return coupling_flip(x, stats, lens, want_next)
 
 
 class Flip(nn.Module):
diff --git a/include/evt.h b/include/evt.h
--- a/include/evt.h
+++ b/include/evt.h
@@ -179,6 +179,24 @@
 int evt_wn_layer_fwd(int32_t dtype, const void* x, const void* w_in_frag, const float* b_in, const void* w_rs_frag,
                      const float* b_rs, const void* g, const void* acc_in, const int32_t* lens, void* x_in, void* acts,
                      void* x_out, void* acc_out, int32_t nseq, int32_t L, int32_t H, int32_t k, int32_t last, void* stream);
+int32_t evt_wn_layer_exit_supported(int32_t dtype, int32_t H, int32_t k, int32_t dil, int32_t cout);
+int32_t evt_wn_layer_entry_supported(int32_t dtype, int32_t H, int32_t k, int32_t dil, int32_t cin, int32_t n_layers);
+int evt_wn_layer_fwd_entry(int32_t dtype, const void* x0, const void* w_entry_frag, const float* b_entry, int32_t cin,
+                           const void* w_in_frag, const float* b_in, const void* w_rs_frag, const float* b_rs, const void* g,
+                           const int32_t* lens, void* h, void* x_in, void* acts, void* x_out, void* acc_out, int32_t nseq,
+                           int32_t L, int32_t H, int32_t k, void* stream);
+int evt_wn_layer_bwd_data_entry(int32_t dtype, const void* dx_next, const void* dacc, const void* x_in, const void* g,
+                                const void* w_rs_alt_frag, const void* w_in_alt_frag, const int32_t* lens, void* drs,
+                                void* dx_in, void* dh, float* dg, const void* w_entry_alt_frag, void* dx0, int32_t nseq,
+                                int32_t L, int32_t H, int32_t k, int32_t cin, void* stream);
+int evt_wn_layer_fwd_exit(int32_t dtype, const void* x, const void* w_in_frag, const float* b_in, const void* w_rs_frag,
+                          const float* b_rs, const void* g, const void* acc_in, const int32_t* lens, void* x_in, void* acts,
+                          void* acc_out, const void* w_exit_frag, const float* b_exit, void* stats, int32_t nseq, int32_t L,
+                          int32_t H, int32_t k, int32_t cout, void* stream);
+int evt_wn_layer_bwd_data_exit(int32_t dtype, const void* dstats, const void* w_exit_alt_frag, const void* x_in, const void* g,
+                               const void* w_rs_alt_frag, const void* w_in_alt_frag, const int32_t* lens, void* drs,
+                               void* dx_in, void* dx, float* dg, int32_t nseq, int32_t L, int32_t H, int32_t k, int32_t cout,
+                               void* stream);
 
 int evt_add3_scale(int32_t dtype, const void* a, const void* b, const void* c, float scale, void* out,
                    int64_t n, void* stream);
```

Result: no change. 3585 audio-s/s, median of 3 (+0.3%).
